# blackjax-devs/blackjax

Measured on NVIDIA B200. Metric: leapfrog-steps/sec (all chains), higher is better.
Workload: dtype f32

## Files before the change

### blackjax_b200/csrc/bjx_dense.cu

```cuda
#include <vector>

#include "bjx_handle.h"
#include "bjx_internal.h"
#include <cuda_fp16.h>

#include "bjx_gemm.h"
#include "bjx_prng.cuh"

using namespace bjx;

namespace bjx {

constexpr int kRowWarps = 8;

__device__ __forceinline__ float wsum(float v) {
#pragma unroll
  for (int o = 16; o > 0; o >>= 1) v += __shfl_xor_sync(0xffffffffu, v, o);
  return v;
}

__device__ __forceinline__ float wmax(float v) {
#pragma unroll
  for (int o = 16; o > 0; o >>= 1) v = fmaxf(v, __shfl_xor_sync(0xffffffffu, v, o));
  return v;
}
__device__ __forceinline__ float max4(float m, float4 v) {
  return fmaxf(fmaxf(m, fmaxf(fabsf(v.x), fabsf(v.y))), fmaxf(fabsf(v.z), fabsf(v.w)));
}

__device__ __forceinline__ void split2(float x, uint16_t& h1, uint16_t& h2) {
  const __half a = __float2half_rn(x);
  const __half b = __float2half_rn(x - __half2float(a));
  h1 = __half_as_ushort(a);
  h2 = __half_as_ushort(b);
}
__device__ __forceinline__ uint2 pack4(const uint16_t (&v)[4]) {
  return make_uint2((uint32_t)v[0] | ((uint32_t)v[1] << 16), (uint32_t)v[2] | ((uint32_t)v[3] << 16));
}
__device__ __forceinline__ void store_planes(uint16_t* row, int KP, int k, float4 v, float sc) {
  uint16_t p1[4], p2[4];
  split2(v.x * sc, p1[0], p2[0]);
  split2(v.y * sc, p1[1], p2[1]);
  split2(v.z * sc, p1[2], p2[2]);
  split2(v.w * sc, p1[3], p2[3]);
  *reinterpret_cast<uint2*>(row + k) = pack4(p1);
  *reinterpret_cast<uint2*>(row + (size_t)KP + k) = pack4(p2);
}

__global__ void k_rows_split2(int R, int K, const float* __restrict__ x, uint16_t* __restrict__ xs, float* __restrict__ unscale,
                              float* __restrict__ rowmax, float* __restrict__ rowmax_zero) {
  const int lane = threadIdx.x & 31, r = blockIdx.x * kRowWarps + (threadIdx.x >> 5);
  if (r >= R) return;
  const float4* xr = reinterpret_cast<const float4*>(x + (size_t)r * K);
  float amax = 0.f;
  for (int i = lane; i < K / 4; i += 32) amax = max4(amax, xr[i]);
  amax = wmax(amax);
  const float sc = pow2_lift(amax);
  const int KP = plane_stride(K);
  uint16_t* row = xs + (size_t)r * 2 * KP;
  for (int i = lane; i < K / 4; i += 32) store_planes(row, KP, 4 * i, xr[i], sc);
  if (lane == 0) {
    unscale[r] = 1.0f / sc;
    if (rowmax) rowmax[r] = amax;
    if (rowmax_zero) rowmax_zero[r] = 0.f;
  }
}

__global__ void k_planes_fixup(int R, int K, const float* __restrict__ y, uint16_t* __restrict__ ys,
                               const float* __restrict__ stale_max, const float* __restrict__ new_max,
                               float* __restrict__ unscale) {
  const int lane = threadIdx.x & 31;
  const int r0 = (blockIdx.x * (blockDim.x >> 5) + (threadIdx.x >> 5)) * 32;
  const int r = r0 + lane;
  asm volatile("griddepcontrol.wait;" ::: "memory");
  bool bad = false;
  if (r < R) {
    const float mx = new_max[r];
    const float t = mx * plane_lift(stale_max[r]);
    bad = (mx > 0.f) && (mx <= 3.0e38f) && !(t >= kPlaneWindowLo && t < kPlaneWindowHi);
  }
  unsigned todo = __ballot_sync(0xffffffffu, bad);
  const int KP = plane_stride(K);
  while (todo) {
    const int rr = r0 + (__ffs(todo) - 1);
    todo &= todo - 1;
    const float sc = pow2_lift(new_max[rr]);
    const float4* xr = reinterpret_cast<const float4*>(y + (size_t)rr * K);
    uint16_t* row = ys + (size_t)rr * 2 * KP;
    for (int i = lane; i < K / 4; i += 32) store_planes(row, KP, 4 * i, xr[i], sc);
    if (lane == 0) unscale[rr] = 1.0f / sc;
  }
}

__global__ void k_absmax(long long n4, const float* __restrict__ x, float* out) {
  float m = 0.f;
  for (long long t = (long long)blockIdx.x * blockDim.x + threadIdx.x; t < n4; t += (long long)gridDim.x * blockDim.x)
    m = max4(m, reinterpret_cast<const float4*>(x)[t]);
  m = wmax(m);
  if ((threadIdx.x & 31) == 0) atomicMax(reinterpret_cast<int*>(out), __float_as_int(m));
}
__global__ void k_matrix_split2(long long R, int K, const float* __restrict__ x, uint16_t* __restrict__ xs,
                                const float* __restrict__ amax, float* __restrict__ unscale) {
  const long long t = (long long)blockIdx.x * blockDim.x + threadIdx.x;
  const float sc = pow2_lift(amax[0]);
  if (t == 0) unscale[0] = 1.0f / sc;
  if (t >= R * K / 4) return;
  const long long e = t * 4;
  const long long r = e / K;
  const int k = (int)(e % K);
  const int KP = plane_stride(K);
  store_planes(xs + r * 2 * KP, KP, k, reinterpret_cast<const float4*>(x)[t], sc);
}

__global__ void k_rows_open(int C, int D, float* __restrict__ p, const float* __restrict__ g, const float* __restrict__ q,
                            float eps, const float* __restrict__ eps_dev, uint16_t* __restrict__ p_planes,
                            float* __restrict__ p_unscale, float* __restrict__ pmax0, float* __restrict__ pmax1,
                            float* __restrict__ qmax0, float* __restrict__ qmax1) {
  const int lane = threadIdx.x & 31, c = blockIdx.x * kRowWarps + (threadIdx.x >> 5);
  if (c >= C) return;
  const size_t ro = (size_t)c * D;
  const float eh = (eps_dev ? eps_dev[c] : eps) * 0.5f;
  float pm = 0.f, qm = 0.f;
  for (int i = lane; i < D / 4; i += 32) {
    float4 pv = __ldcs(reinterpret_cast<const float4*>(p + ro) + i);
    const float4 gv = __ldcs(reinterpret_cast<const float4*>(g + ro) + i);
    pv.x = fmaf(eh, gv.x, pv.x); pv.y = fmaf(eh, gv.y, pv.y); pv.z = fmaf(eh, gv.z, pv.z); pv.w = fmaf(eh, gv.w, pv.w);
    reinterpret_cast<float4*>(p + ro)[i] = pv;
    pm = max4(pm, pv);
    if (q) qm = max4(qm, __ldcs(reinterpret_cast<const float4*>(q + ro) + i));
  }
  pm = wmax(pm);
  qm = wmax(qm);
  const float sc = pow2_lift(pm);
  const int KP = plane_stride(D);
  uint16_t* row = p_planes + (size_t)c * 2 * KP;
  for (int i = lane; i < D / 4; i += 32) store_planes(row, KP, 4 * i, reinterpret_cast<const float4*>(p + ro)[i], sc);
  if (lane == 0) {
    p_unscale[c] = 1.0f / sc;
    pmax0[c] = pm;
    pmax1[c] = 0.f;
    if (q) { qmax0[c] = qm; qmax1[c] = 0.f; }
  }
}

__global__ void k_dense_normal(int C, int D, const uint32_t* __restrict__ keys, float* __restrict__ z, bool split_first,
                               int key_shared, uint32_t chain_offset) {
  const long long t = (long long)blockIdx.x * blockDim.x + threadIdx.x;
  const long long n4 = (long long)C * D / 4;
  if (t >= n4) return;
  const long long e = t * 4;
  const int c = (int)(e / D);
  const uint32_t i = (uint32_t)(e % D);
  Key km = key_shared ? fold_in(Key{keys[0], keys[1]}, chain_offset + (uint32_t)c) : Key{keys[2 * c], keys[2 * c + 1]};
  if (split_first) km = fold_in(km, 0u);
  float4 o;
  o.x = normal_at(km, i);
  o.y = normal_at(km, i + 1);
  o.z = normal_at(km, i + 2);
  o.w = normal_at(km, i + 3);
  reinterpret_cast<float4*>(z)[t] = o;
}

__global__ void k_rows_scale(int C, int D, const float* __restrict__ a, long long a_stride, const float* __restrict__ x,
                             float* __restrict__ y) {
  const long long t = (long long)blockIdx.x * blockDim.x + threadIdx.x;
  const long long n4 = (long long)C * D / 4;
  if (t >= n4) return;
  const long long e = t * 4;
  const int c = (int)(e / D);
  const int i = (int)(e % D);
  const float4 av = *reinterpret_cast<const float4*>(a + (size_t)c * a_stride + i);
  const float4 xv = __ldcs(reinterpret_cast<const float4*>(x) + t);
  __stcs(reinterpret_cast<float4*>(y) + t, make_float4(av.x * xv.x, av.y * xv.y, av.z * xv.z, av.w * xv.w));
}

__global__ void k_rows_axpy(int C, int D, float* __restrict__ x, const float* __restrict__ y, float eps,
                            const float* __restrict__ eps_dev, float coef) {
  const long long t = (long long)blockIdx.x * blockDim.x + threadIdx.x;
  const long long n4 = (long long)C * D / 4;
  if (t >= n4) return;
  const int c = (int)(t * 4 / D);
  const float a = (eps_dev ? eps_dev[c] : eps) * coef;
  float4 xv = __ldcs(reinterpret_cast<const float4*>(x) + t);
  const float4 yv = __ldcs(reinterpret_cast<const float4*>(y) + t);
  xv.x = fmaf(a, yv.x, xv.x); xv.y = fmaf(a, yv.y, xv.y); xv.z = fmaf(a, yv.z, xv.z); xv.w = fmaf(a, yv.w, xv.w);
  __stcs(reinterpret_cast<float4*>(x) + t, xv);
}

__global__ void k_rows_energy(int C, int D, const float* __restrict__ v, const float* __restrict__ p,
                              const float* __restrict__ logp, float* __restrict__ e, float p_sign) {
  const int lane = threadIdx.x & 31, c = blockIdx.x * kRowWarps + (threadIdx.x >> 5);
  if (c >= C) return;
  const float4* vr = reinterpret_cast<const float4*>(v + (size_t)c * D);
  const float4* pr = reinterpret_cast<const float4*>(p + (size_t)c * D);
  float acc = 0.f;
  for (int i = lane; i < D / 4; i += 32) {
    const float4 a = __ldcs(vr + i), b = __ldcs(pr + i);
    acc = fmaf(a.x, b.x, acc); acc = fmaf(a.y, b.y, acc); acc = fmaf(a.z, b.z, acc); acc = fmaf(a.w, b.w, acc);
  }
  acc = wsum(acc);
  if (lane == 0) e[c] = -logp[c] + 0.5f * acc * p_sign;
}

template <int TARGET>
__global__ void k_rows_grad_kick(int C, int D, const float* __restrict__ q, const float* __restrict__ aux,
                                 const float* __restrict__ inv_var, const float* __restrict__ mean, float offset,
                                 float* __restrict__ p, float eps, const float* __restrict__ eps_dev,
                                 float* __restrict__ g_out, float* __restrict__ logp_out, int kicks,
                                 uint16_t* __restrict__ p_split ,
                                 float* __restrict__ p_unscale) {
  const int lane = threadIdx.x & 31, c = blockIdx.x * kRowWarps + (threadIdx.x >> 5);
  if (c >= C) return;
  const size_t ro = (size_t)c * D;
  const float eps_c = eps_dev ? eps_dev[c] : eps;
  const float eh = eps_c * 0.5f;
  float acc = 0.f, amax = 0.f;
  for (int i = lane; i < D / 4; i += 32) {
    const float4 qv = __ldcs(reinterpret_cast<const float4*>(q + ro) + i);
    float4 gv;
    if (TARGET == 2) {
      gv = __ldcs(reinterpret_cast<const float4*>(aux + ro) + i);
      acc = fmaf(qv.x, gv.x, acc); acc = fmaf(qv.y, gv.y, acc); acc = fmaf(qv.z, gv.z, acc); acc = fmaf(qv.w, gv.w, acc);
    } else {
      const float4 w = __ldg(reinterpret_cast<const float4*>(inv_var) + i);
      float4 d = qv;
      if (mean) {
        const float4 m = __ldg(reinterpret_cast<const float4*>(mean) + i);
        d = make_float4(qv.x - m.x, qv.y - m.y, qv.z - m.z, qv.w - m.w);
      }
      gv = make_float4(d.x * -w.x, d.y * -w.y, d.z * -w.z, d.w * -w.w);
      acc = fmaf(d.x, gv.x, acc); acc = fmaf(d.y, gv.y, acc); acc = fmaf(d.z, gv.z, acc); acc = fmaf(d.w, gv.w, acc);
    }
    if (TARGET != 2) __stcs(reinterpret_cast<float4*>(g_out + ro) + i, gv);
    if (p) {
      float4 pv = __ldcs(reinterpret_cast<const float4*>(p + ro) + i);
      pv.x = fmaf(eh, gv.x, pv.x); pv.y = fmaf(eh, gv.y, pv.y); pv.z = fmaf(eh, gv.z, pv.z); pv.w = fmaf(eh, gv.w, pv.w);
      if (kicks == 2) {
        pv.x = fmaf(eh, gv.x, pv.x); pv.y = fmaf(eh, gv.y, pv.y); pv.z = fmaf(eh, gv.z, pv.z); pv.w = fmaf(eh, gv.w, pv.w);
      }
      if (p_split) {
        reinterpret_cast<float4*>(p + ro)[i] = pv;
        amax = max4(amax, pv);
      } else {
        __stcs(reinterpret_cast<float4*>(p + ro) + i, pv);
      }
    }
  }
  if (p_split) {
    const float sc = pow2_lift(wmax(amax));
    const int KP = plane_stride(D);
    uint16_t* row = p_split + (size_t)c * 2 * KP;
    for (int i = lane; i < D / 4; i += 32) store_planes(row, KP, 4 * i, reinterpret_cast<const float4*>(p + ro)[i], sc);
    if (lane == 0) p_unscale[c] = 1.0f / sc;
  }
  acc = wsum(acc);
  if (lane == 0) logp_out[c] = 0.5f * acc + offset;
}

__global__ void k_rows_accept(int C, int D, const uint32_t* __restrict__ keys, const float* __restrict__ e0,
                              const float* __restrict__ e1, float div_thr, const float* __restrict__ qw,
                              const float* __restrict__ gw, const float* __restrict__ lw, const float* q_in,
                              const float* g_in, const float* l_in, float* q_out, float* g_out, float* l_out, int L,
                              InfoPtrs info, int key_shared, uint32_t chain_offset) {
  const int lane = threadIdx.x & 31, c = blockIdx.x * kRowWarps + (threadIdx.x >> 5);
  if (c >= C) return;
  const Key rk = key_shared ? fold_in(Key{keys[0], keys[1]}, chain_offset + (uint32_t)c) : Key{keys[2 * c], keys[2 * c + 1]};
  const Key ki = fold_in(rk, 1u);
  float delta = e0[c] - e1[c];
  if (isnan(delta)) delta = -__int_as_float(0x7f800000);
  const bool is_div = (-delta) > div_thr;
  float pa = expf(delta);
  pa = pa > 1.0f ? 1.0f : pa;
  const bool acc = uniform01(ki) < pa;
  const size_t ro = (size_t)c * D;
  if (acc || q_out != q_in) {
    const float4* sq = reinterpret_cast<const float4*>((acc ? qw : q_in) + ro);
    const float4* sg = reinterpret_cast<const float4*>((acc ? gw : g_in) + ro);
    for (int i = lane; i < D / 4; i += 32) {
      __stcs(reinterpret_cast<float4*>(q_out + ro) + i, __ldcs(sq + i));
      __stcs(reinterpret_cast<float4*>(g_out + ro) + i, __ldcs(sg + i));
    }
    if (lane == 0) l_out[c] = acc ? lw[c] : l_in[c];
  }
  if (lane == 0) {
    if (info.acceptance_rate) info.acceptance_rate[c] = pa;
    if (info.is_accepted) info.is_accepted[c] = acc;
    if (info.is_divergent) info.is_divergent[c] = is_div;
    if (info.energy) info.energy[c] = e1[c];
    if (info.num_integration_steps) info.num_integration_steps[c] = L;
  }
}
}

#define DN_CUDA(call)                                                \
  do {                                                               \
    cudaError_t e_ = (call);                                         \
    if (e_ != cudaSuccess) return bjx_cuda_fail(h, e_, #call);       \
  } while (0)
#define DN_LAUNCH(where)                                             \
  do {                                                               \
    cudaError_t e_ = cudaGetLastError();                             \
    if (e_ != cudaSuccess) return bjx_cuda_fail(h, e_, where);       \
  } while (0)

static inline dim3 g4(long long n4) { return dim3((unsigned)((n4 + 255) / 256)); }
static inline dim3 grow(int C) { return dim3((C + kRowWarps - 1) / kRowWarps); }

struct DenseWs {
  float *p, *v, *q, *g, *lw, *e0, *e1;
  uint16_t* xs[2];
  float* unscale[2];
  float* rmax[2];
  float* mat_max;
  float* mat_unscale;
};
enum { MAT_IMM = 0, MAT_MSQRT = 1, MAT_PREC = 2 };
enum { PL_P = 0, PL_Q = 1 };

constexpr int kParts = 1;
struct Part {
  int c0, n;
  cudaStream_t st;
  int index;
};

static int dense_ws(bjx_handle_t h, DenseWs& w) {
  const size_t C = h->cfg.n_chains, D = h->cfg.dim;
  const size_t row = ((C * D * sizeof(float)) + 255) & ~(size_t)255, vec = ((C * sizeof(float)) + 255) & ~(size_t)255;
  const size_t KP = plane_stride((int)D);
  const size_t xsb = ((C * 2 * KP * sizeof(uint16_t)) + 255) & ~(size_t)255;
  const size_t mat = ((D * 2 * KP * sizeof(uint16_t)) + 255) & ~(size_t)255;
  const size_t need = 4 * row + 11 * vec + 2 * xsb + 3 * mat + 256;
  if (h->dense_bytes < need) {
    if (h->dense_block) DN_CUDA(cudaFree(h->dense_block));
    h->dense_block = nullptr;
    DN_CUDA(cudaMalloc((void**)&h->dense_block, need));
    h->dense_bytes = need;
  }
  if (!h->dense_streams_ready) {
    for (int k = 0; k < 2; ++k) {
      DN_CUDA(cudaStreamCreateWithFlags(&h->dense_stream[k], cudaStreamNonBlocking));
      DN_CUDA(cudaEventCreateWithFlags(&h->dense_join[k], cudaEventDisableTiming));
    }
    DN_CUDA(cudaEventCreateWithFlags(&h->dense_fork, cudaEventDisableTiming));
    DN_CUDA(cudaEventCreateWithFlags(&h->dense_stagger, cudaEventDisableTiming));
    h->dense_streams_ready = true;
  }
  char* b = (char*)h->dense_block;
  w.p = (float*)b; w.v = (float*)(b + row); w.q = (float*)(b + 2 * row); w.g = (float*)(b + 3 * row);
  char* vb = b + 4 * row;
  w.lw = (float*)vb; w.e0 = (float*)(vb + vec); w.e1 = (float*)(vb + 2 * vec);
  w.unscale[PL_P] = (float*)(vb + 3 * vec); w.unscale[PL_Q] = (float*)(vb + 4 * vec);
  w.rmax[PL_P] = (float*)(vb + 5 * vec); w.rmax[PL_Q] = (float*)(vb + 8 * vec);
  char* xb = vb + 11 * vec;
  w.xs[PL_P] = (uint16_t*)xb; w.xs[PL_Q] = (uint16_t*)(xb + xsb);
  for (int m = 0; m < 3; ++m) h->dense_mat_s[m] = (uint16_t*)(xb + 2 * xsb + m * mat);
  w.mat_max = (float*)(xb + 2 * xsb + 3 * mat);
  w.mat_unscale = w.mat_max + 4;
  if (h->dense_bytes_built != need) {
    DN_CUDA(cudaMemsetAsync(vb, 0, 11 * vec + 2 * xsb + 3 * mat, h->stream));
    for (int m = 0; m < 3; ++m) h->dense_mat_src[m] = nullptr;
    h->dense_bytes_built = need;
  }
  const float* src[3] = {h->metric_kind == BJX_METRIC_DENSE ? h->imm : nullptr,
                         h->metric_kind == BJX_METRIC_DENSE ? h->msqrt : nullptr,
                         h->cfg.target.kind == BJX_TARGET_DENSE_GAUSSIAN ? h->cfg.target.precision : nullptr};
  for (int m = 0; m < 3; ++m) {
    if (src[m] && (h->dense_mat_src[m] != src[m] || h->dense_mat_ver[m] != h->dense_version)) {
      DN_CUDA(cudaMemsetAsync(w.mat_max + m, 0, sizeof(float), h->stream));
      k_absmax<<<148, 256, 0, h->stream>>>((long long)D * D / 4, src[m], w.mat_max + m);
      DN_LAUNCH("k_absmax");
      k_matrix_split2<<<g4((long long)D * D / 4), 256, 0, h->stream>>>((long long)D, (int)D, src[m], h->dense_mat_s[m],
                                                                      w.mat_max + m, w.mat_unscale + m);
      DN_LAUNCH("k_matrix_split2");
      h->dense_mat_src[m] = src[m];
      h->dense_mat_ver[m] = h->dense_version;
    }
  }
  return 0;
}

template <class F>
static int for_parts(bjx_handle_t h, F fn) {
  const int C = h->cfg.n_chains;
  const int parts = (C >= 8192) ? kParts : 1;
  if (parts == 1) {
    Part pt{0, C, h->stream, -1};
    return fn(pt);
  }
  DN_CUDA(cudaEventRecord(h->dense_fork, h->stream));
  int rc = 0;
  for (int k = 0; k < parts; ++k) {
    const int c0 = (int)((long long)C * k / parts) & ~255, c1 = (k + 1 == parts) ? C : ((int)((long long)C * (k + 1) / parts) & ~255);
    Part pt{c0, c1 - c0, h->dense_stream[k], k};
    DN_CUDA(cudaStreamWaitEvent(pt.st, h->dense_fork, 0));
    if (rc == 0) rc = fn(pt);
    DN_CUDA(cudaEventRecord(h->dense_join[k], pt.st));
    DN_CUDA(cudaStreamWaitEvent(h->stream, h->dense_join[k], 0));
  }
  return rc;
}

struct PlanesOut {
  int var;
  int phase;
};

static int gemm(bjx_handle_t h, DenseWs& w, const Part& pt, const float* X, int xvar, int mat, float* Y, const float* Cin,
                float alpha, const float* alpha_dev, float beta, bool double_kick = false, PlanesOut po = PlanesOut{-1, 0}) {
  const int D = h->cfg.dim, C = h->cfg.n_chains;
  const size_t ro = (size_t)pt.c0 * D;
  const int KP = plane_stride(D);
  uint16_t* xs = w.xs[xvar] + (size_t)pt.c0 * 2 * KP;
  if (X) {
    k_rows_split2<<<grow(pt.n), kRowWarps * 32, 0, pt.st>>>(pt.n, D, X + ro, xs, w.unscale[xvar] + pt.c0, nullptr, nullptr);
    DN_LAUNCH("k_rows_split2");
  }
  GemmCall g;
  g.x_planes = xs;
  g.a_planes = h->dense_mat_s[mat];
  g.Y = Y + ro;
  g.Cin = Cin ? Cin + ro : nullptr;
  g.planes_out = nullptr;
  g.M = pt.n; g.N = D; g.K = D; g.KP = KP; g.KP_out = KP;
  g.epi.alpha = alpha;
  g.epi.alpha_dev = alpha_dev ? alpha_dev + pt.c0 : nullptr;
  g.epi.x_unscale = w.unscale[xvar] + pt.c0;
  g.epi.mat_unscale = w.mat_unscale + mat;
  g.epi.beta = beta;
  g.epi.has_cin = Cin ? 1 : 0;
  g.epi.double_kick = double_kick ? 1 : 0;
  g.epi.planes = 0;
  g.epi.debug = 0;
  g.epi.out_unscale = nullptr; g.epi.stale_max = nullptr; g.epi.next_max = nullptr; g.epi.zero_max = nullptr;
  if (po.var >= 0) {
    float* ring = w.rmax[po.var];
    g.planes_out = w.xs[po.var] + (size_t)pt.c0 * 2 * KP;
    g.epi.planes = 1;
    g.epi.out_unscale = w.unscale[po.var] + pt.c0;
    g.epi.stale_max = ring + (size_t)(po.phase % 3) * C + pt.c0;
    g.epi.next_max = ring + (size_t)((po.phase + 1) % 3) * C + pt.c0;
    g.epi.zero_max = ring + (size_t)((po.phase + 2) % 3) * C + pt.c0;
  }
  const int rc = gemm_f16x3(g, pt.st);
  if (rc) return bjx_fail(h, BJX_E_UNSUPPORTED, "tensor-core product failed (stage " + std::to_string(rc) + ")");
  if (po.var >= 0) {
    cudaLaunchConfig_t cfg = {};
    cfg.gridDim = dim3((pt.n + 255) / 256);
    cfg.blockDim = dim3(256);
    cfg.stream = pt.st;
    cudaLaunchAttribute attr[1];
    attr[0].id = cudaLaunchAttributeProgrammaticStreamSerialization;
    attr[0].val.programmaticStreamSerializationAllowed = 1;
    cfg.attrs = attr;
    cfg.numAttrs = 1;
    DN_CUDA(cudaLaunchKernelEx(&cfg, k_planes_fixup, pt.n, D, (const float*)(Y + ro), g.planes_out, g.epi.stale_max,
                               (const float*)g.epi.next_max, g.epi.out_unscale));
  }
  return 0;
}

static int dense_velocity(bjx_handle_t h, DenseWs& w, const Part& pt, const float* p, float* v, bool p_presplit = false) {
  const int D = h->cfg.dim;
  if (h->metric_kind == BJX_METRIC_DENSE) return gemm(h, w, pt, p_presplit ? nullptr : p, PL_P, MAT_IMM, v, nullptr, 1.f, nullptr, 0.f);
  const bool per_chain = (h->metric_kind == BJX_METRIC_DIAG_PER_CHAIN);
  const size_t ro = (size_t)pt.c0 * D;
  k_rows_scale<<<g4((long long)pt.n * D / 4), 256, 0, pt.st>>>(pt.n, D, h->imm + (per_chain ? ro : 0), per_chain ? D : 0,
                                                              p + ro, v + ro);
  DN_LAUNCH("k_rows_scale");
  return 0;
}

static int dense_grad(bjx_handle_t h, DenseWs& w, const Part& pt, const float* q, float* p, float eps, const float* eps_dev,
                      float* g, float* logp, int kicks = 1, bool split_p = false, bool q_presplit = false) {
  const int D = h->cfg.dim;
  const bjx_target_desc& t = h->cfg.target;
  const size_t ro = (size_t)pt.c0 * D;
  const float* ed = eps_dev ? eps_dev + pt.c0 : nullptr;
  float* pp = p ? p + ro : nullptr;
  uint16_t* ps = (split_p && pp) ? w.xs[PL_P] + (size_t)pt.c0 * 2 * plane_stride(D) : nullptr;
  if (t.kind == BJX_TARGET_DENSE_GAUSSIAN) {
    int rc = gemm(h, w, pt, q_presplit ? nullptr : q, PL_Q, MAT_PREC, g, nullptr, -1.f, nullptr, 0.f);
    if (rc) return rc;
    k_rows_grad_kick<2><<<grow(pt.n), kRowWarps * 32, 0, pt.st>>>(pt.n, D, q + ro, g + ro, nullptr, nullptr, t.logp_offset,
                                                                pp, eps, ed, g + ro, logp + pt.c0, kicks, ps,
                                                                w.unscale[PL_P] + pt.c0);
  } else if (t.kind == BJX_TARGET_DIAG_GAUSSIAN) {
    k_rows_grad_kick<0><<<grow(pt.n), kRowWarps * 32, 0, pt.st>>>(pt.n, D, q + ro, nullptr, t.inv_var, t.mean, t.logp_offset,
                                                                pp, eps, ed, g + ro, logp + pt.c0, kicks, ps,
                                                                w.unscale[PL_P] + pt.c0);
  } else {
    return bjx_fail(h, BJX_E_UNSUPPORTED, "large-D dense path supports DENSE_GAUSSIAN and DIAG_GAUSSIAN targets");
  }
  DN_LAUNCH("k_rows_grad_kick");
  return 0;
}

static int dense_momentum(bjx_handle_t h, DenseWs& w, const Part& pt, const uint32_t* keys, float* p_out, bool split_first) {
  const int D = h->cfg.dim;
  const size_t ro = (size_t)pt.c0 * D;
  const bool dense_m = (h->metric_kind == BJX_METRIC_DENSE);
  float* z = dense_m ? w.v : p_out;
  const uint32_t* kp = h->key_shared ? keys : keys + 2 * (size_t)pt.c0;
  k_dense_normal<<<g4((long long)pt.n * D / 4), 256, 0, pt.st>>>(pt.n, D, kp, z + ro, split_first, h->key_shared,
                                                                h->chain_offset + (uint32_t)pt.c0);
  DN_LAUNCH("k_dense_normal");
  if (dense_m) return gemm(h, w, pt, z, PL_P, MAT_MSQRT, p_out, nullptr, 1.f, nullptr, 0.f);
  const bool per_chain = (h->metric_kind == BJX_METRIC_DIAG_PER_CHAIN);
  k_rows_scale<<<g4((long long)pt.n * D / 4), 256, 0, pt.st>>>(pt.n, D, h->msqrt + (per_chain ? ro : 0), per_chain ? D : 0,
                                                              z + ro, p_out + ro);
  DN_LAUNCH("k_rows_scale");
  return 0;
}

static int dense_energy(bjx_handle_t h, DenseWs& w, const Part& pt, const float* p, const float* logp, float* e_out,
                        bool p_presplit = false) {
  const int D = h->cfg.dim;
  int rc = dense_velocity(h, w, pt, p, w.v, p_presplit);
  if (rc) return rc;
  const size_t ro = (size_t)pt.c0 * D;
  k_rows_energy<<<grow(pt.n), kRowWarps * 32, 0, pt.st>>>(pt.n, D, w.v + ro, p + ro, logp + pt.c0, e_out + pt.c0, 1.f);
  DN_LAUNCH("k_rows_energy");
  return 0;
}

static int dense_leapfrog_core(bjx_handle_t h, DenseWs& w, const Part& pt, float* q, float* p, float* logp, float* g,
                               float eps, const float* eps_dev, int n_steps, bool p_planes_after = false) {
  const int D = h->cfg.dim, C = h->cfg.n_chains;
  const long long n4 = (long long)pt.n * D / 4;
  const size_t ro = (size_t)pt.c0 * D;
  const float* ed = eps_dev ? eps_dev + pt.c0 : nullptr;
  const bool dense_m = (h->metric_kind == BJX_METRIC_DENSE);
  const bool dense_t = (h->cfg.target.kind == BJX_TARGET_DENSE_GAUSSIAN);
  if (n_steps <= 0) return 0;
  if (dense_m && dense_t) {
    const int KP = plane_stride(D);
    float *pr = w.rmax[PL_P] + pt.c0, *qr = w.rmax[PL_Q] + pt.c0;
    k_rows_open<<<grow(pt.n), kRowWarps * 32, 0, pt.st>>>(pt.n, D, p + ro, g + ro, q + ro, eps, ed,
                                                         w.xs[PL_P] + (size_t)pt.c0 * 2 * KP, w.unscale[PL_P] + pt.c0, pr, pr + C,
                                                         qr, qr + C);
    DN_LAUNCH("k_rows_open");
    int pphase = 0, qphase = 0;
    for (int s = 0; s < n_steps; ++s) {
      int rc = gemm(h, w, pt, nullptr, PL_P, MAT_IMM, q, q, eps_dev ? 1.0f : eps * 1.0f, eps_dev, 1.f, false, PlanesOut{PL_Q, qphase++});
      if (rc) return rc;
      if (s + 1 < n_steps) {
        rc = gemm(h, w, pt, nullptr, PL_Q, MAT_PREC, p, p, eps_dev ? -0.5f : -(eps * 0.5f), eps_dev, 1.f, true, PlanesOut{PL_P, pphase++});
        if (rc) return rc;
      } else {
        rc = dense_grad(h, w, pt, q, p, eps, eps_dev, g, logp, 1, p_planes_after, true);
        if (rc) return rc;
      }
    }
    return 0;
  }
  k_rows_axpy<<<g4(n4), 256, 0, pt.st>>>(pt.n, D, p + ro, g + ro, eps, ed, 0.5f);
  DN_LAUNCH("k_rows_axpy");
  bool p_presplit = false;
  for (int s = 0; s < n_steps; ++s) {
    int rc;
    if (dense_m) {
      rc = gemm(h, w, pt, p_presplit ? nullptr : p, PL_P, MAT_IMM, q, q, eps_dev ? 1.0f : eps * 1.0f, eps_dev, 1.f);
      if (rc) return rc;
    } else {
      rc = dense_velocity(h, w, pt, p, w.v);
      if (rc) return rc;
      k_rows_axpy<<<g4(n4), 256, 0, pt.st>>>(pt.n, D, q + ro, w.v + ro, eps, ed, 1.0f);
      DN_LAUNCH("k_rows_axpy");
    }
    const bool more = (s + 1 < n_steps);
    const bool want_planes = dense_m && (more || p_planes_after);
    rc = dense_grad(h, w, pt, q, p, eps, eps_dev, g, logp, more ? 2 : 1, want_planes);
    if (rc) return rc;
    p_presplit = want_planes;
  }
  return 0;
}

int bjx_dense_velocity(bjx_handle_t h, const float* p, float* v) {
  DenseWs w;
  int rc = dense_ws(h, w);
  if (rc) return rc;
  return for_parts(h, [&](const Part& pt) { return dense_velocity(h, w, pt, p, v); });
}

int bjx_dense_init_state(bjx_handle_t h, const float* q, float* logp_out, float* grad_out) {
  DenseWs w;
  int rc = dense_ws(h, w);
  if (rc) return rc;
  return for_parts(h, [&](const Part& pt) { return dense_grad(h, w, pt, q, nullptr, 0.f, nullptr, grad_out, logp_out); });
}

int bjx_dense_sample_momentum(bjx_handle_t h, const uint32_t* keys, float* p_out, bool split_first) {
  DenseWs w;
  int rc = dense_ws(h, w);
  if (rc) return rc;
  return for_parts(h, [&](const Part& pt) { return dense_momentum(h, w, pt, keys, p_out, split_first); });
}

int bjx_dense_energy(bjx_handle_t h, const float* p, const float* logp, float* e_out) {
  DenseWs w;
  int rc = dense_ws(h, w);
  if (rc) return rc;
  return for_parts(h, [&](const Part& pt) { return dense_energy(h, w, pt, p, logp, e_out); });
}

int bjx_dense_leapfrog(bjx_handle_t h, float* q, float* p, float* logp, float* g, float eps, const float* eps_dev,
                       int n_steps) {
  DenseWs w;
  int rc = dense_ws(h, w);
  if (rc) return rc;
  return for_parts(h, [&](const Part& pt) { return dense_leapfrog_core(h, w, pt, q, p, logp, g, eps, eps_dev, n_steps); });
}

static int dense_hmc_part(bjx_handle_t h, DenseWs& w, const Part& pt, const uint32_t* keys, const float* q_in,
                          const float* logp_in, const float* g_in, float* q_out, float* logp_out, float* g_out, float eps,
                          const float* eps_dev, int L, const InfoPtrs& info) {
  const int D = h->cfg.dim;
  const size_t ro = (size_t)pt.c0 * D;
  const size_t bytes = (size_t)pt.n * D * sizeof(float);
  int rc = dense_momentum(h, w, pt, keys, w.p, true);
  if (rc) return rc;
  if (info.momentum) DN_CUDA(cudaMemcpyAsync(info.momentum + ro, w.p + ro, bytes, cudaMemcpyDeviceToDevice, pt.st));
  rc = dense_energy(h, w, pt, w.p, logp_in, w.e0);
  if (rc) return rc;
  DN_CUDA(cudaMemcpyAsync(w.q + ro, q_in + ro, bytes, cudaMemcpyDeviceToDevice, pt.st));
  DN_CUDA(cudaMemcpyAsync(w.g + ro, g_in + ro, bytes, cudaMemcpyDeviceToDevice, pt.st));
  DN_CUDA(cudaMemcpyAsync(w.lw + pt.c0, logp_in + pt.c0, (size_t)pt.n * sizeof(float), cudaMemcpyDeviceToDevice, pt.st));
  const bool planes_after = (h->metric_kind == BJX_METRIC_DENSE) && L > 0;
  rc = dense_leapfrog_core(h, w, pt, w.q, w.p, w.lw, w.g, eps, eps_dev, L, planes_after);
  if (rc) return rc;
  rc = dense_energy(h, w, pt, w.p, w.lw, w.e1, planes_after);
  if (rc) return rc;
  if (info.proposal_position) DN_CUDA(cudaMemcpyAsync(info.proposal_position + ro, w.q + ro, bytes, cudaMemcpyDeviceToDevice, pt.st));
  if (info.proposal_momentum) {
    DN_CUDA(cudaMemsetAsync(info.proposal_momentum + ro, 0, bytes, pt.st));
    k_rows_axpy<<<g4((long long)pt.n * D / 4), 256, 0, pt.st>>>(pt.n, D, info.proposal_momentum + ro, w.p + ro, -1.0f, nullptr, 1.0f);
    DN_LAUNCH("k_rows_axpy");
  }
  InfoPtrs ip = info;
  if (ip.acceptance_rate) ip.acceptance_rate += pt.c0;
  if (ip.is_accepted) ip.is_accepted += pt.c0;
  if (ip.is_divergent) ip.is_divergent += pt.c0;
  if (ip.energy) ip.energy += pt.c0;
  if (ip.num_integration_steps) ip.num_integration_steps += pt.c0;
  const uint32_t* kp = h->key_shared ? keys : keys + 2 * (size_t)pt.c0;
  k_rows_accept<<<grow(pt.n), kRowWarps * 32, 0, pt.st>>>(pt.n, D, kp, w.e0 + pt.c0, w.e1 + pt.c0, h->cfg.divergence_threshold,
                                                         w.q + ro, w.g + ro, w.lw + pt.c0, q_in + ro, g_in + ro, logp_in + pt.c0,
                                                         q_out + ro, g_out + ro, logp_out + pt.c0, L, ip, h->key_shared,
                                                         h->chain_offset + (uint32_t)pt.c0);
  DN_LAUNCH("k_rows_accept");
  return 0;
}

int bjx_dense_hmc_step(bjx_handle_t h, const uint32_t* keys, const float* q_in, const float* logp_in, const float* g_in,
                       float* q_out, float* logp_out, float* g_out, float eps, const float* eps_dev, int L,
                       const InfoPtrs& info) {
  DenseWs w;
  int rc = dense_ws(h, w);
  if (rc) return rc;
  return for_parts(h, [&](const Part& pt) {
    return dense_hmc_part(h, w, pt, keys, q_in, logp_in, g_in, q_out, logp_out, g_out, eps, eps_dev, L, info);
  });
}

#include "bjx_dense_nuts.cuh"
```

### blackjax_b200/csrc/bjx_dense_nuts.cuh

```cuda
namespace bjx {

struct DnWs {
  float *cq, *cp, *cg, *cv, *cps;
  float *ck_p, *ck_s, *ck_v;
  float *left_v, *right_v;
  float *clogp, *ceps, *sub_weight, *sub_slpa, *sub_logp, *sub_energy, *u_prop;
  int *cn, *cdone, *cdir;
  uint32_t* ctk;
};

__device__ __forceinline__ float dn_dot(const float* a, const float* b, int D, int lane) {
  float acc = 0.f;
  for (int i = lane; i < D / 4; i += 32) {
    const float4 x = reinterpret_cast<const float4*>(a)[i], y = reinterpret_cast<const float4*>(b)[i];
    acc = fmaf(x.x, y.x, acc); acc = fmaf(x.y, y.y, acc); acc = fmaf(x.z, y.z, acc); acc = fmaf(x.w, y.w, acc);
  }
  return wsum(acc);
}
__device__ __forceinline__ void dn_copy(float* dst, const float* src, int D, int lane) {
  for (int i = lane; i < D / 4; i += 32) reinterpret_cast<float4*>(dst)[i] = reinterpret_cast<const float4*>(src)[i];
}
__device__ __forceinline__ void dn_kick(float* p, const float* g, float eh, int D, int lane, uint16_t* planes, float* unscale) {
  float amax = 0.f;
  for (int i = lane; i < D / 4; i += 32) {
    float4 pv = reinterpret_cast<const float4*>(p)[i];
    const float4 gv = reinterpret_cast<const float4*>(g)[i];
    pv.x = fmaf(eh, gv.x, pv.x); pv.y = fmaf(eh, gv.y, pv.y); pv.z = fmaf(eh, gv.z, pv.z); pv.w = fmaf(eh, gv.w, pv.w);
    reinterpret_cast<float4*>(p)[i] = pv;
    amax = max4(amax, pv);
  }
  if (planes) {
    const float sc = pow2_lift(wmax(amax));
    const int KP = plane_stride(D);
    for (int i = lane; i < D / 4; i += 32) store_planes(planes, KP, 4 * i, reinterpret_cast<const float4*>(p)[i], sc);
    if (lane == 0) *unscale = 1.0f / sc;
  }
}
__device__ __forceinline__ bool dn_turning(const float* pl, const float* vl, const float* pr, const float* vr, const float* psum,
                                           const float* sub_a, const float* sub_b, int D, int lane) {
  float al = 0.f, ar = 0.f;
  for (int i = lane; i < D / 4; i += 32) {
    const float4 a = reinterpret_cast<const float4*>(pl)[i], b = reinterpret_cast<const float4*>(pr)[i];
    float4 s = reinterpret_cast<const float4*>(psum)[i];
    if (sub_a) {
      const float4 x = reinterpret_cast<const float4*>(sub_a)[i], y = reinterpret_cast<const float4*>(sub_b)[i];
      s = make_float4(s.x - x.x + y.x, s.y - x.y + y.y, s.z - x.z + y.z, s.w - x.w + y.w);
    }
    const float4 u = reinterpret_cast<const float4*>(vl)[i], w = reinterpret_cast<const float4*>(vr)[i];
    const float r0 = s.x - (b.x + a.x) / 2.0f, r1 = s.y - (b.y + a.y) / 2.0f, r2 = s.z - (b.z + a.z) / 2.0f,
                r3 = s.w - (b.w + a.w) / 2.0f;
    al = fmaf(u.x, r0, al); al = fmaf(u.y, r1, al); al = fmaf(u.z, r2, al); al = fmaf(u.w, r3, al);
    ar = fmaf(w.x, r0, ar); ar = fmaf(w.y, r1, ar); ar = fmaf(w.z, r2, ar); ar = fmaf(w.w, r3, ar);
  }
  al = wsum(al);
  ar = wsum(ar);
  return (al <= 0.f) || (ar <= 0.f);
}

__global__ void k_dn_init(int C, int D, NutsWs ws, DnWs dn, const uint32_t* __restrict__ keys, int key_shared,
                          uint32_t chain_offset, const uint32_t* __restrict__ keyint_override, const float* q_in,
                          const float* logp_in, const float* g_in, float* q_out, float* logp_out, float* g_out, float* mom_out) {
  const int lane = threadIdx.x & 31, c = blockIdx.x * kRowWarps + (threadIdx.x >> 5);
  if (c >= C) return;
  const size_t ro = (size_t)c * D;
  const float kin = 0.5f * dn_dot(dn.left_v + ro, ws.left_p + ro, D, lane);
  dn_copy(ws.right_p + ro, ws.left_p + ro, D, lane);
  dn_copy(dn.right_v + ro, dn.left_v + ro, D, lane);
  dn_copy(ws.psum + ro, ws.left_p + ro, D, lane);
  dn_copy(ws.left_q + ro, q_in + ro, D, lane);
  dn_copy(ws.right_q + ro, q_in + ro, D, lane);
  dn_copy(ws.left_g + ro, g_in + ro, D, lane);
  dn_copy(ws.right_g + ro, g_in + ro, D, lane);
  if (mom_out) dn_copy(mom_out + ro, ws.left_p + ro, D, lane);
  if (q_out != q_in) {
    dn_copy(q_out + ro, q_in + ro, D, lane);
    dn_copy(g_out + ro, g_in + ro, D, lane);
  }
  if (lane == 0) {
    const float logp0 = logp_in[c];
    const float h0 = -logp0 + kin;
    Key ki;
    if (keyint_override) {
      ki = Key{keyint_override[2 * c], keyint_override[2 * c + 1]};
    } else {
      const Key rk = key_shared ? fold_in(Key{keys[0], keys[1]}, chain_offset + (uint32_t)c) : Key{keys[2 * c], keys[2 * c + 1]};
      ki = fold_in(rk, 1u);
    }
    if (q_out != q_in) logp_out[c] = logp0;
    ws.left_logp[c] = logp0;
    ws.right_logp[c] = logp0;
    ws.h0[c] = h0;
    ws.prop_energy[c] = h0;
    ws.prop_weight[c] = 0.f;
    ws.prop_slpa[c] = -__int_as_float(0x7f800000);
    ws.n_states[c] = 0;
    ws.step[c] = 0;
    ws.is_div[c] = 0;
    ws.is_turn[c] = 0;
    ws.key_int[2 * c] = ki.a;
    ws.key_int[2 * c + 1] = ki.b;
  }
}

__global__ void k_dn_begin(int n, int D, int d, NutsWs ws, DnWs dn, const int* __restrict__ list, float eps,
                           const float* __restrict__ eps_dev, uint16_t* __restrict__ p_planes, float* __restrict__ p_unscale) {
  const int lane = threadIdx.x & 31, r = blockIdx.x * kRowWarps + (threadIdx.x >> 5);
  if (r >= n) return;
  const int c = list ? list[r] : r;
  const size_t ro = (size_t)c * D, rr = (size_t)r * D;
  const Key ki{ws.key_int[2 * c], ws.key_int[2 * c + 1]};
  const Key sub = fold_in(ki, (uint32_t)d);
  const int dir = (uniform01(fold_in(sub, 0u)) < 0.5f) ? 1 : -1;
  const Key tk = fold_in(sub, 1u);
  const float ec = (float)dir * (eps_dev ? eps_dev[c] : eps);
  dn_copy(dn.cq + rr, (dir > 0 ? ws.right_q : ws.left_q) + ro, D, lane);
  dn_copy(dn.cp + rr, (dir > 0 ? ws.right_p : ws.left_p) + ro, D, lane);
  dn_copy(dn.cg + rr, (dir > 0 ? ws.right_g : ws.left_g) + ro, D, lane);
  __syncwarp();
  dn_kick(dn.cp + rr, dn.cg + rr, ec * 0.5f, D, lane, p_planes ? p_planes + (size_t)r * 2 * plane_stride(D) : nullptr,
          p_unscale + r);
  if (lane == 0) {
    dn.cdir[r] = dir;
    dn.ceps[r] = ec;
    dn.ctk[2 * r] = tk.a;
    dn.ctk[2 * r + 1] = tk.b;
    dn.u_prop[r] = uniform01(fold_in(sub, 2u));
    dn.cn[r] = 0;
    dn.cdone[r] = 0;
    dn.sub_weight[r] = -__int_as_float(0x7f800000);
    dn.sub_slpa[r] = -__int_as_float(0x7f800000);
    dn.sub_logp[r] = 0.f;
    dn.sub_energy[r] = 0.f;
  }
}

__global__ void k_dn_leaf(int n, int D, int i, int last, int C, NutsWs ws, DnWs dn, const int* __restrict__ list, float div_thr,
                          uint16_t* __restrict__ p_planes, float* __restrict__ p_unscale) {
  const int lane = threadIdx.x & 31, r = blockIdx.x * kRowWarps + (threadIdx.x >> 5);
  if (r >= n) return;
  if (dn.cdone[r]) return;
  const int c = list ? list[r] : r;
  const size_t ro = (size_t)c * D, rr = (size_t)r * D;
  const float* p = dn.cp + rr;
  const float* v = dn.cv + rr;
  float* ps = dn.cps + rr;
  const float logp = dn.clogp[r];
  const float e_new = -logp + 0.5f * dn_dot(v, p, D, lane);
  const float w_new = safe_energy_diff(ws.h0[c], e_new);
  const float slpa_new = fminf(w_new, 0.f);
  const bool is_div = (-w_new) > div_thr;
  float sub_weight = dn.sub_weight[r], sub_slpa = dn.sub_slpa[r];
  bool take;
  if (i == 0) {
    dn_copy(ps, p, D, lane);
    take = true;
    sub_weight = w_new;
    sub_slpa = slpa_new;
  } else {
    for (int k = lane; k < D / 4; k += 32) {
      float4 a = reinterpret_cast<float4*>(ps)[k];
      const float4 b = reinterpret_cast<const float4*>(p)[k];
      a.x = a.x + b.x; a.y = a.y + b.y; a.z = a.z + b.z; a.w = a.w + b.w;
      reinterpret_cast<float4*>(ps)[k] = a;
    }
    const Key tk{dn.ctk[2 * r], dn.ctk[2 * r + 1]};
    const float u_leaf = uniform01(fold_in(tk, (uint32_t)i));
    take = u_leaf < expit_f(w_new - sub_weight);
    sub_weight = logaddexp_f(sub_weight, w_new);
    sub_slpa = logaddexp_f(sub_slpa, slpa_new);
  }
  __syncwarp();
  if (take) {
    dn_copy(ws.sub_prop_q + ro, dn.cq + rr, D, lane);
    dn_copy(ws.sub_prop_g + ro, dn.cg + rr, D, lane);
  }
  const int idx_max = __popc((unsigned)i >> 1);
  const int idx_min = idx_max - __popc((~(unsigned)i & ((unsigned)i + 1u)) - 1u) + 1;
  const size_t lvl = (size_t)C * D;
  if ((i & 1) == 0) {
    dn_copy(dn.ck_p + idx_max * lvl + rr, p, D, lane);
    dn_copy(dn.ck_s + idx_max * lvl + rr, ps, D, lane);
    dn_copy(dn.ck_v + idx_max * lvl + rr, v, D, lane);
  }
  __syncwarp();
  bool turning = false;
  for (int k = idx_max; k >= idx_min && !turning; --k)
    turning = dn_turning(dn.ck_p + k * lvl + rr, dn.ck_v + k * lvl + rr, p, v, ps, dn.ck_s + k * lvl + rr, dn.ck_p + k * lvl + rr,
                         D, lane);
  const bool stop = is_div || turning;
  const int dir = dn.cdir[r];
  if (stop || i == last) {
    dn_copy((dir > 0 ? ws.right_q : ws.left_q) + ro, dn.cq + rr, D, lane);
    dn_copy((dir > 0 ? ws.right_p : ws.left_p) + ro, p, D, lane);
    dn_copy((dir > 0 ? ws.right_g : ws.left_g) + ro, dn.cg + rr, D, lane);
    dn_copy((dir > 0 ? dn.right_v : dn.left_v) + ro, v, D, lane);
  } else {
    __syncwarp();
    dn_kick(dn.cp + rr, dn.cg + rr, dn.ceps[r] * 0.5f, D, lane,
            p_planes ? p_planes + (size_t)r * 2 * plane_stride(D) : nullptr, p_unscale + r);
  }
  if (lane == 0) {
    dn.sub_weight[r] = sub_weight;
    dn.sub_slpa[r] = sub_slpa;
    if (take) {
      dn.sub_logp[r] = logp;
      dn.sub_energy[r] = e_new;
    }
    dn.cn[r] = i + 1;
    if (stop || i == last) {
      if (dir > 0) ws.right_logp[c] = logp; else ws.left_logp[c] = logp;
    }
    if (stop) dn.cdone[r] = is_div ? 1 : 2;
    if (stop && is_div && turning) dn.cdone[r] = 3;
  }
}

__global__ void k_dn_end(int n, int D, int d, int max_doublings, NutsWs ws, DnWs dn, const int* __restrict__ list,
                         int* __restrict__ list_out, int* __restrict__ counter_out, float* q_out, float* logp_out, float* g_out) {
  const int lane = threadIdx.x & 31, r = blockIdx.x * kRowWarps + (threadIdx.x >> 5);
  if (r >= n) return;
  const int c = list ? list[r] : r;
  const size_t ro = (size_t)c * D, rr = (size_t)r * D;
  const int done = dn.cdone[r];
  const bool sub_div = (done & 1) != 0, sub_term = (done & 2) != 0;
  const bool bad = sub_div || sub_term;
  const float sub_weight = dn.sub_weight[r];
  float prop_weight = ws.prop_weight[c];
  bool take2 = false;
  if (!bad) take2 = dn.u_prop[r] < clip_max1(expf(sub_weight - prop_weight));
  if (take2) {
    dn_copy(q_out + ro, ws.sub_prop_q + ro, D, lane);
    dn_copy(g_out + ro, ws.sub_prop_g + ro, D, lane);
  }
  for (int k = lane; k < D / 4; k += 32) {
    float4 a = reinterpret_cast<float4*>(ws.psum + ro)[k];
    const float4 b = reinterpret_cast<const float4*>(dn.cps + rr)[k];
    a.x = a.x + b.x; a.y = a.y + b.y; a.z = a.z + b.z; a.w = a.w + b.w;
    reinterpret_cast<float4*>(ws.psum + ro)[k] = a;
  }
  __syncwarp();
  const bool turning = dn_turning(ws.left_p + ro, dn.left_v + ro, ws.right_p + ro, dn.right_v + ro, ws.psum + ro, nullptr, nullptr,
                                  D, lane);
  const bool is_turn = sub_term || turning;
  const bool run_next = (d + 1 < max_doublings) && !sub_div && !is_turn;
  if (lane == 0) {
    if (!bad) prop_weight = logaddexp_f(prop_weight, sub_weight);
    ws.prop_weight[c] = prop_weight;
    ws.prop_slpa[c] = logaddexp_f(ws.prop_slpa[c], dn.sub_slpa[r]);
    ws.n_states[c] += dn.cn[r];
    ws.step[c] = d + 1;
    if (take2) {
      logp_out[c] = dn.sub_logp[r];
      ws.prop_energy[c] = dn.sub_energy[r];
    }
    ws.is_div[c] = sub_div;
    ws.is_turn[c] = is_turn;
    if (run_next) list_out[atomicAdd(counter_out, 1)] = c;
  }
}

static int dn_ws(bjx_handle_t h, DnWs& dn) {
  const size_t C = h->cfg.n_chains, D = h->cfg.dim, depth = h->cfg.max_tree_depth;
  const size_t row = ((C * D * sizeof(float)) + 255) & ~(size_t)255, vec = ((C * sizeof(float)) + 255) & ~(size_t)255;
  const size_t need = (7 + depth) * row + 12 * vec + 256;
  if (h->dn_bytes < need) {
    if (h->dn_block) DN_CUDA(cudaFree(h->dn_block));
    h->dn_block = nullptr;
    DN_CUDA(cudaMalloc(&h->dn_block, need));
    h->dn_bytes = need;
  }
  char* b = (char*)h->dn_block;
  auto take = [&](size_t bytes) { char* r = b; b += bytes; return r; };
  dn.cq = (float*)take(row); dn.cp = (float*)take(row); dn.cg = (float*)take(row); dn.cv = (float*)take(row);
  dn.cps = (float*)take(row); dn.left_v = (float*)take(row); dn.right_v = (float*)take(row);
  dn.ck_v = (float*)take(depth * row);
  dn.ck_p = h->ws.ckpt_p;
  dn.ck_s = h->ws.ckpt_sum;
  dn.clogp = (float*)take(vec); dn.ceps = (float*)take(vec); dn.sub_weight = (float*)take(vec); dn.sub_slpa = (float*)take(vec);
  dn.sub_logp = (float*)take(vec); dn.sub_energy = (float*)take(vec); dn.u_prop = (float*)take(vec);
  dn.cn = (int*)take(vec); dn.cdone = (int*)take(vec); dn.cdir = (int*)take(vec);
  dn.ctk = (uint32_t*)take(2 * vec);
  return 0;
}

}

using namespace bjx;

int bjx_dense_nuts_step(bjx_handle_t h, const uint32_t* keys, const float* q_in, const float* logp_in, const float* g_in,
                        float* q_out, float* logp_out, float* g_out, float step_size, const float* step_size_dev,
                        int max_num_doublings, InfoPtrs info, const float* momentum_override,
                        const uint32_t* key_integrator_override) {
  DN_CUDA(cudaSetDevice(h->cfg.device));
  const int C = h->cfg.n_chains, D = h->cfg.dim;
  int rc = bjx_ensure_nuts_ws(h);
  if (rc) return rc;
  DenseWs w;
  rc = dense_ws(h, w);
  if (rc) return rc;
  DnWs dn;
  rc = dn_ws(h, dn);
  if (rc) return rc;
  NutsWs& ws = h->ws;
  cudaStream_t st = h->stream;
  const bool dense_m = (h->metric_kind == BJX_METRIC_DENSE);
  Part all{0, C, st, -1};
  DN_CUDA(cudaMemsetAsync(ws.counters, 0, 64 * sizeof(int), st));
  if (momentum_override) {
    DN_CUDA(cudaMemcpyAsync(ws.left_p, momentum_override, (size_t)C * D * sizeof(float), cudaMemcpyDeviceToDevice, st));
  } else {
    rc = dense_momentum(h, w, all, keys, ws.left_p, true);
    if (rc) return rc;
  }
  rc = dense_velocity(h, w, all, ws.left_p, dn.left_v);
  if (rc) return rc;
  k_dn_init<<<grow(C), kRowWarps * 32, 0, st>>>(C, D, ws, dn, keys, h->key_shared, h->chain_offset, key_integrator_override, q_in,
                                                logp_in, g_in, q_out, logp_out, g_out, info.momentum);
  DN_LAUNCH("k_dn_init");

  int n = C;
  const int* list = nullptr;
  int64_t launches = 0;
  for (int d = 0; d < max_num_doublings && n > 0; ++d) {
    Part pt{0, n, st, -1};
    uint16_t* planes = dense_m ? w.xs[PL_P] : nullptr;
    k_dn_begin<<<grow(n), kRowWarps * 32, 0, st>>>(n, D, d, ws, dn, list, step_size, step_size_dev, planes, w.unscale[PL_P]);
    DN_LAUNCH("k_dn_begin");
    const int leaves = 1 << d;
    for (int i = 0; i < leaves; ++i) {
      rc = dense_velocity(h, w, pt, dn.cp, w.v, dense_m);
      if (rc) return rc;
      k_rows_axpy<<<g4((long long)n * D / 4), 256, 0, st>>>(n, D, dn.cq, w.v, 0.f, dn.ceps, 1.0f);
      DN_LAUNCH("k_rows_axpy");
      rc = dense_grad(h, w, pt, dn.cq, dn.cp, 0.f, dn.ceps, dn.cg, dn.clogp, 1, dense_m, false);
      if (rc) return rc;
      rc = dense_velocity(h, w, pt, dn.cp, dn.cv, dense_m);
      if (rc) return rc;
      k_dn_leaf<<<grow(n), kRowWarps * 32, 0, st>>>(n, D, i, leaves - 1, C, ws, dn, list, h->cfg.divergence_threshold, planes,
                                                    w.unscale[PL_P]);
      DN_LAUNCH("k_dn_leaf");
      ++launches;
    }
    int* list_out = (d & 1) ? ws.list_b : ws.list_a;
    k_dn_end<<<grow(n), kRowWarps * 32, 0, st>>>(n, D, d, max_num_doublings, ws, dn, list, list_out, ws.counters + 1 + d, q_out,
                                                 logp_out, g_out);
    DN_LAUNCH("k_dn_end");
    if (d + 1 < max_num_doublings) {
      DN_CUDA(cudaMemcpyAsync(h->h_flag, ws.counters + 1 + d, sizeof(int), cudaMemcpyDeviceToHost, st));
      DN_CUDA(cudaStreamSynchronize(st));
      n = h->h_flag[0];
      list = list_out;
    }
  }
  k_nuts_finish<<<(C + 255) / 256, 256, 0, st>>>(C, ws, info);
  DN_LAUNCH("k_nuts_finish");
  h->last_leaf_launches = launches;
  h->last_depth = -1;
  return 0;
}
```

### blackjax_b200/csrc/bjx_gemm.cu

```cuda
#include <cuda.h>
#include <cuda_fp16.h>
#include <cuda_runtime.h>
#include <stdint.h>

#include <cstdlib>
#include <mutex>

#include "bjx_gemm.h"

namespace bjx {
namespace {

constexpr int kBM = 128;
constexpr int kBN = 256;
constexpr int kUmmaK = 16;
constexpr int kSub = 32;
constexpr int kNSub = kBN / kSub;
constexpr int kThreads = 256;
constexpr uint32_t kTmemCols = 512;
constexpr int kYSlab = 32 * kSub * 4;
constexpr int kPSlab = 32 * kSub * 2;

template <int BK, int STAGES, int NY, int NP>
struct Plan {
  static constexpr int kTileBytes = kBM * BK * 2;
  static constexpr int kStageBytes = 4 * kTileBytes;
  static constexpr int kOffY = STAGES * kStageBytes;
  static constexpr int kOffP = kOffY + 4 * NY * kYSlab;
  static constexpr int kOffBar = kOffP + 4 * NP * 2 * kPSlab;
  static constexpr int kNumBars = 2 * STAGES + 4 + 4 * NY;
  static constexpr int kSmemBytes = kOffBar + kNumBars * 8 + 16 + 1024;
  static_assert(kSmemBytes <= 232448, "over the 227 KB dynamic shared memory limit");
  static_assert(BK == 64 || BK == 32, "one swizzle row per tile row: 128-byte or 64-byte swizzle");
};

__device__ __forceinline__ uint32_t smem_u32(const void* p) { return (uint32_t)__cvta_generic_to_shared(p); }
__device__ __forceinline__ uint32_t cluster_ctarank() {
  uint32_t r;
  asm volatile("mov.u32 %0, %%cluster_ctarank;" : "=r"(r));
  return r;
}
__device__ __forceinline__ uint32_t mapa(uint32_t addr, uint32_t rank) {
  uint32_t r;
  asm volatile("mapa.shared::cluster.u32 %0, %1, %2;" : "=r"(r) : "r"(addr), "r"(rank));
  return r;
}
__device__ __forceinline__ void cluster_sync() {
  asm volatile("barrier.cluster.arrive.release.aligned;\n\tbarrier.cluster.wait.acquire.aligned;" ::: "memory");
}
__device__ __forceinline__ void mbar_init(uint32_t bar, uint32_t count) {
  asm volatile("mbarrier.init.shared::cta.b64 [%0], %1;" ::"r"(bar), "r"(count) : "memory");
}
__device__ __forceinline__ void mbar_wait(uint32_t bar, uint32_t parity) {
  uint32_t done;
  do {
    asm volatile(
        "{\n\t.reg .pred p;\n\t"
        "mbarrier.try_wait.parity.shared::cta.b64 p, [%1], %2;\n\t"
        "selp.u32 %0, 1, 0, p;\n\t}"
        : "=r"(done)
        : "r"(bar), "r"(parity)
        : "memory");
  } while (!done);
}
__device__ __forceinline__ void mbar_wait_cluster(uint32_t bar, uint32_t parity) {
  uint32_t done;
  do {
    asm volatile(
        "{\n\t.reg .pred p;\n\t"
        "mbarrier.try_wait.parity.acquire.cluster.shared::cta.b64 p, [%1], %2;\n\t"
        "selp.u32 %0, 1, 0, p;\n\t}"
        : "=r"(done)
        : "r"(bar), "r"(parity)
        : "memory");
  } while (!done);
}
__device__ __forceinline__ void mbar_expect_tx(uint32_t bar, uint32_t bytes) {
  asm volatile("mbarrier.arrive.expect_tx.shared::cta.b64 _, [%0], %1;" ::"r"(bar), "r"(bytes) : "memory");
}
__device__ __forceinline__ void mbar_arrive_cluster(uint32_t cluster_bar) {
  asm volatile("mbarrier.arrive.release.cluster.shared::cluster.b64 _, [%0];" ::"r"(cluster_bar) : "memory");
}
__device__ __forceinline__ void prefetch_tmap(const CUtensorMap* m) {
  asm volatile("prefetch.tensormap [%0];" ::"l"(reinterpret_cast<uint64_t>(m)) : "memory");
}
__device__ __forceinline__ void tma_load_3d_2sm(uint32_t dst, const CUtensorMap* m, uint32_t leader_bar, int c0, int c1, int c2) {
  asm volatile(
      "cp.async.bulk.tensor.3d.cta_group::2.shared::cluster.global.mbarrier::complete_tx::bytes [%0], [%1, {%3, %4, %5}], [%2];"
      ::"r"(dst), "l"(reinterpret_cast<uint64_t>(m)), "r"(leader_bar), "r"(c0), "r"(c1), "r"(c2)
      : "memory");
}
__device__ __forceinline__ void tma_load_2d(uint32_t dst, const CUtensorMap* m, uint32_t bar, int c0, int c1) {
  asm volatile(
      "cp.async.bulk.tensor.2d.shared::cluster.global.mbarrier::complete_tx::bytes [%0], [%1, {%3, %4}], [%2];"
      ::"r"(dst), "l"(reinterpret_cast<uint64_t>(m)), "r"(bar), "r"(c0), "r"(c1)
      : "memory");
}
__device__ __forceinline__ void tma_store_2d(const CUtensorMap* m, uint32_t src, int c0, int c1) {
  asm volatile("cp.async.bulk.tensor.2d.global.shared::cta.bulk_group [%0, {%2, %3}], [%1];" ::"l"(reinterpret_cast<uint64_t>(m)),
               "r"(src), "r"(c0), "r"(c1)
               : "memory");
}
__device__ __forceinline__ void tma_store_3d(const CUtensorMap* m, uint32_t src, int c0, int c1, int c2) {
  asm volatile("cp.async.bulk.tensor.3d.global.shared::cta.bulk_group [%0, {%2, %3, %4}], [%1];" ::"l"(reinterpret_cast<uint64_t>(m)),
               "r"(src), "r"(c0), "r"(c1), "r"(c2)
               : "memory");
}
__device__ __forceinline__ void tma_store_commit() { asm volatile("cp.async.bulk.commit_group;" ::: "memory"); }
template <int N>
__device__ __forceinline__ void tma_store_wait_read() { asm volatile("cp.async.bulk.wait_group.read %0;" ::"n"(N) : "memory"); }
__device__ __forceinline__ void tma_store_wait_all() { asm volatile("cp.async.bulk.wait_group 0;" ::: "memory"); }
__device__ __forceinline__ void fence_proxy_async() { asm volatile("fence.proxy.async.shared::cta;" ::: "memory"); }
__device__ __forceinline__ void tc_fence_before() { asm volatile("tcgen05.fence::before_thread_sync;" ::: "memory"); }
__device__ __forceinline__ void tc_fence_after() { asm volatile("tcgen05.fence::after_thread_sync;" ::: "memory"); }

__device__ __forceinline__ void umma_f16_2sm(uint32_t tmem_d, uint64_t desc_a, uint64_t desc_b, uint32_t idesc, uint32_t accumulate) {
  asm volatile(
      "{\n\t.reg .pred p;\n\t"
      "setp.ne.b32 p, %4, 0;\n\t"
      "tcgen05.mma.cta_group::2.kind::f16 [%0], %1, %2, %3, p;\n\t}"
      ::"r"(tmem_d), "l"(desc_a), "l"(desc_b), "r"(idesc), "r"(accumulate)
      : "memory");
}
__device__ __forceinline__ void umma_commit_2sm(uint32_t bar) {
  asm volatile("tcgen05.commit.cta_group::2.mbarrier::arrive::one.shared::cluster.multicast::cluster.b64 [%0], %1;" ::"r"(bar),
               "h"((uint16_t)3)
               : "memory");
}
__device__ __forceinline__ void tmem_ld32(uint32_t taddr, uint32_t (&v)[32]) {
  asm volatile(
      "tcgen05.ld.sync.aligned.32x32b.x32.b32 "
      "{%0, %1, %2, %3, %4, %5, %6, %7, %8, %9, %10, %11, %12, %13, %14, %15, "
      "%16, %17, %18, %19, %20, %21, %22, %23, %24, %25, %26, %27, %28, %29, %30, %31}, [%32];"
      : "=r"(v[0]), "=r"(v[1]), "=r"(v[2]), "=r"(v[3]), "=r"(v[4]), "=r"(v[5]), "=r"(v[6]), "=r"(v[7]), "=r"(v[8]), "=r"(v[9]),
        "=r"(v[10]), "=r"(v[11]), "=r"(v[12]), "=r"(v[13]), "=r"(v[14]), "=r"(v[15]), "=r"(v[16]), "=r"(v[17]), "=r"(v[18]),
        "=r"(v[19]), "=r"(v[20]), "=r"(v[21]), "=r"(v[22]), "=r"(v[23]), "=r"(v[24]), "=r"(v[25]), "=r"(v[26]), "=r"(v[27]),
        "=r"(v[28]), "=r"(v[29]), "=r"(v[30]), "=r"(v[31])
      : "r"(taddr)
      : "memory");
}
__device__ __forceinline__ void tmem_ld_wait() { asm volatile("tcgen05.wait::ld.sync.aligned;" ::: "memory"); }
__device__ __forceinline__ float4 lds_f4(uint32_t a) {
  float4 v;
  asm volatile("ld.shared.v4.f32 {%0, %1, %2, %3}, [%4];" : "=f"(v.x), "=f"(v.y), "=f"(v.z), "=f"(v.w) : "r"(a));
  return v;
}
__device__ __forceinline__ void sts_f4(uint32_t a, float4 v) {
  asm volatile("st.shared.v4.f32 [%0], {%1, %2, %3, %4};" ::"r"(a), "f"(v.x), "f"(v.y), "f"(v.z), "f"(v.w) : "memory");
}
__device__ __forceinline__ void sts_u4(uint32_t a, uint32_t x, uint32_t y, uint32_t z, uint32_t w) {
  asm volatile("st.shared.v4.b32 [%0], {%1, %2, %3, %4};" ::"r"(a), "r"(x), "r"(y), "r"(z), "r"(w) : "memory");
}

template <int BK>
__device__ __forceinline__ uint64_t umma_desc(uint32_t smem_addr) {
  const uint32_t lo = ((smem_addr & 0x3FFFFu) >> 4) | (1u << 16);
  const uint32_t hi = ((8u * BK * 2u) >> 4) | (1u << 14) | ((BK == 64 ? 2u : 4u) << 29);
  return (uint64_t)lo | ((uint64_t)hi << 32);
}
constexpr uint32_t kIdesc = (1u << 4) | ((uint32_t)(kBN >> 3) << 17) | ((uint32_t)(256 >> 4) << 24);

__device__ __forceinline__ uint32_t pack_h2(float a, float b) {
  const __half2 h = __floats2half2_rn(a, b);
  return *reinterpret_cast<const uint32_t*>(&h);
}
__device__ __forceinline__ float2 unpack_h2(uint32_t u) { return __half22float2(*reinterpret_cast<const __half2*>(&u)); }

}

__device__ unsigned long long g_gemm_prof[16];
__device__ __forceinline__ unsigned long long clk() {
  unsigned long long t;
  asm volatile("mov.u64 %0, %%clock64;" : "=l"(t));
  return t;
}
#define BJX_PROF_BEGIN(var) unsigned long long var = prof ? clk() : 0ull
#define BJX_PROF_END(var, acc) \
  if (prof) acc += clk() - var

template <int BK, int STAGES, int NY, int NP>
__global__ void __cluster_dims__(2, 1, 1) __launch_bounds__(kThreads, 1)
k_gemm_f16x3(const __grid_constant__ CUtensorMap tm_x,
             const __grid_constant__ CUtensorMap tm_a,
             const __grid_constant__ CUtensorMap tm_c,
             const __grid_constant__ CUtensorMap tm_y,
             const __grid_constant__ CUtensorMap tm_p,
             const GemmEpilogue E, const int M, const int N, const int K, const int tiles_n, const int n_tiles) {
  using P = Plan<BK, STAGES, NY, NP>;
  extern __shared__ uint8_t smem_raw[];
  const uint32_t base = (smem_u32(smem_raw) + 1023u) & ~1023u;
  const uint32_t bar0 = base + P::kOffBar;
  auto full_bar = [&](int s) { return bar0 + 8u * s; };
  auto empty_bar = [&](int s) { return bar0 + 8u * (STAGES + s); };
  auto tfull_bar = [&](int a) { return bar0 + 8u * (2 * STAGES + a); };
  auto tempty_bar = [&](int a) { return bar0 + 8u * (2 * STAGES + 2 + a); };
  auto cin_bar = [&](int q, int slot) { return bar0 + 8u * (2 * STAGES + 4 + q * NY + slot); };
  const uint32_t tmem_slot = bar0 + 8u * P::kNumBars;

  const int warp = threadIdx.x >> 5, lane = threadIdx.x & 31;
  const uint32_t rank = cluster_ctarank();
  const int pair = blockIdx.x >> 1, n_pairs = gridDim.x >> 1;
  const int nkb = (K + BK - 1) / BK;
  const bool prof = (E.debug & 16) != 0;

  if (warp == 0 && lane == 0) {
    prefetch_tmap(&tm_x);
    prefetch_tmap(&tm_a);
    prefetch_tmap(&tm_y);
    if (E.has_cin) prefetch_tmap(&tm_c);
    if (E.planes) prefetch_tmap(&tm_p);
  }
  if (warp == 1 && lane == 0) {
    for (int s = 0; s < STAGES; ++s) {
      mbar_init(full_bar(s), 1);
      mbar_init(empty_bar(s), 1);
    }
    for (int a = 0; a < 2; ++a) {
      mbar_init(tfull_bar(a), 1);
      mbar_init(tempty_bar(a), 8);
    }
    for (int q = 0; q < 4; ++q)
      for (int i = 0; i < NY; ++i) mbar_init(cin_bar(q, i), 1);
    asm volatile("fence.mbarrier_init.release.cluster;" ::: "memory");
  }
  if (warp == 2) {
    asm volatile("tcgen05.alloc.cta_group::2.sync.aligned.shared::cta.b32 [%0], %1;" ::"r"(tmem_slot), "r"(kTmemCols) : "memory");
    asm volatile("tcgen05.relinquish_alloc_permit.cta_group::2.sync.aligned;" ::: "memory");
  }
  tc_fence_before();
  cluster_sync();
  tc_fence_after();
  uint32_t tmem_base;
  asm volatile("ld.shared.u32 %0, [%1];" : "=r"(tmem_base) : "r"(tmem_slot));
  asm volatile("griddepcontrol.wait;" ::: "memory");

  if (warp == 0) {
    if (lane == 0) {
      const uint32_t leader_full0 = mapa(full_bar(0), 0);
      int s = 0;
      uint32_t ph = 0;
      unsigned long long w_empty = 0;
      for (int t = pair; t < n_tiles; t += n_pairs) {
        const int m0 = (t / tiles_n) * (2 * kBM) + (int)rank * kBM;
        const int n0 = (t % tiles_n) * kBN + (int)rank * (kBN / 2);
        for (int kb = 0; kb < nkb; ++kb) {
          BJX_PROF_BEGIN(t0);
          mbar_wait(empty_bar(s), ph ^ 1u);
          BJX_PROF_END(t0, w_empty);
          if (rank == 0) mbar_expect_tx(full_bar(s), 2u * P::kStageBytes);
          const uint32_t st = base + (uint32_t)s * P::kStageBytes;
          const uint32_t fb = leader_full0 + 8u * s;
          tma_load_3d_2sm(st, &tm_x, fb, kb * BK, 0, m0);
          tma_load_3d_2sm(st + 2 * P::kTileBytes, &tm_a, fb, kb * BK, 0, n0);
          tma_load_3d_2sm(st + P::kTileBytes, &tm_x, fb, kb * BK, 1, m0);
          tma_load_3d_2sm(st + 3 * P::kTileBytes, &tm_a, fb, kb * BK, 1, n0);
          if (++s == STAGES) { s = 0; ph ^= 1u; }
        }
      }
      if (prof) atomicAdd(&g_gemm_prof[3], w_empty);
      for (int i = 0; i < STAGES; ++i) {
        mbar_wait(empty_bar(s), ph ^ 1u);
        if (++s == STAGES) { s = 0; ph ^= 1u; }
      }
    }
  } else if (warp == 1) {
    if (rank == 0 && lane == 0) {
      int s = 0, as = 0;
      uint32_t ph = 0, aph = 0;
      unsigned long long w_tempty = 0, w_full = 0;
      BJX_PROF_BEGIN(t_all);
      for (int t = pair; t < n_tiles; t += n_pairs) {
        BJX_PROF_BEGIN(t0);
        mbar_wait_cluster(tempty_bar(as), aph ^ 1u);
        BJX_PROF_END(t0, w_tempty);
        tc_fence_after();
        const uint32_t d = tmem_base + (uint32_t)as * kBN;
        for (int kb = 0; kb < nkb; ++kb) {
          BJX_PROF_BEGIN(t1);
          mbar_wait(full_bar(s), ph);
          BJX_PROF_END(t1, w_full);
          tc_fence_after();
          const uint32_t st = base + (uint32_t)s * P::kStageBytes;
          const uint64_t dx1 = umma_desc<BK>(st), dx2 = umma_desc<BK>(st + P::kTileBytes);
          const uint64_t da1 = umma_desc<BK>(st + 2 * P::kTileBytes), da2 = umma_desc<BK>(st + 3 * P::kTileBytes);
#pragma unroll
          for (int k = 0; k < BK / kUmmaK; ++k)
            umma_f16_2sm(d, dx1 + 2u * k, da1 + 2u * k, kIdesc, (kb | k) != 0);
#pragma unroll
          for (int k = 0; k < BK / kUmmaK; ++k) umma_f16_2sm(d, dx2 + 2u * k, da1 + 2u * k, kIdesc, 1u);
#pragma unroll
          for (int k = 0; k < BK / kUmmaK; ++k) umma_f16_2sm(d, dx1 + 2u * k, da2 + 2u * k, kIdesc, 1u);
          umma_commit_2sm(empty_bar(s));
          if (++s == STAGES) { s = 0; ph ^= 1u; }
        }
        umma_commit_2sm(tfull_bar(as));
        if (++as == 2) { as = 0; aph ^= 1u; }
      }
      if (prof) {
        atomicAdd(&g_gemm_prof[0], w_tempty);
        atomicAdd(&g_gemm_prof[1], w_full);
        atomicAdd(&g_gemm_prof[2], clk() - t_all);
        atomicAdd(&g_gemm_prof[9], 1ull);
      }
    }
  } else if (warp >= 4) {
    const int q = warp & 3;
    const uint32_t ybuf = base + P::kOffY + (uint32_t)q * NY * kYSlab;
    const uint32_t pbuf = base + P::kOffP + (uint32_t)q * NP * 2 * kPSlab;
    const uint32_t leader_tempty0 = mapa(tempty_bar(0), 0);
    const float mat_unscale = E.mat_unscale ? E.mat_unscale[0] : 1.0f;
    const int my_tiles = pair < n_tiles ? (n_tiles - pair + n_pairs - 1) / n_pairs : 0;
    const int n_sub = my_tiles * kNSub;
    const int row_off = (int)rank * kBM + q * 32;
    auto sub_n = [&](int i) { return ((pair + (i / kNSub) * n_pairs) % tiles_n) * kBN + (i % kNSub) * kSub; };
    auto sub_m = [&](int i) { return ((pair + (i / kNSub) * n_pairs) / tiles_n) * (2 * kBM) + row_off; };
    auto load_cin = [&](int i) {
      const uint32_t bar = cin_bar(q, i % NY);
      if (sub_n(i) >= N || (E.debug & 1)) {
        asm volatile("mbarrier.arrive.shared::cta.b64 _, [%0];" ::"r"(bar) : "memory");
        return;
      }
      mbar_expect_tx(bar, kYSlab);
      tma_load_2d(ybuf + (uint32_t)(i % NY) * kYSlab, &tm_c, bar, sub_n(i), sub_m(i));
    };
    constexpr int kAhead = NY - NP;
    if (E.has_cin && lane == 0)
      for (int i = 0; i < kAhead && i < n_sub; ++i) load_cin(i);

    int as = 0;
    uint32_t aph = 0;
    unsigned long long w_tfull = 0, w_cin = 0, w_rd = 0, w_work = 0;
    BJX_PROF_BEGIN(t_all);
    float al = 0.f, sc = 1.f, amax = 0.f;
    int r = 0;
    bool live = false;
    uint32_t tacc = 0;
    for (int i = 0; i < n_sub; ++i) {
      const int j = i % kNSub;
      const int n0s = sub_n(i), m0s = sub_m(i);
      if (lane == 0) {
        BJX_PROF_BEGIN(t0);
        tma_store_wait_read<NP - 1>();
        BJX_PROF_END(t0, w_rd);
        if (E.has_cin && i + kAhead < n_sub) load_cin(i + kAhead);
      }
      __syncwarp();
      if (j == 0) {
        r = m0s + lane;
        live = r < M;
        al = E.alpha;
        if (live) {
          if (E.alpha_dev) al = E.alpha_dev[r] * E.alpha;
          al = al * (E.x_unscale ? E.x_unscale[r] : 1.0f) * mat_unscale;
        }
        sc = 1.0f;
        if (E.planes && live) sc = plane_lift(E.stale_max[r]);
        amax = 0.f;
        BJX_PROF_BEGIN(t0);
        mbar_wait(tfull_bar(as), aph);
        BJX_PROF_END(t0, w_tfull);
        tc_fence_after();
        tacc = tmem_base + (uint32_t)as * kBN + ((uint32_t)(q * 32) << 16);
      }
      uint32_t acc[32];
      tmem_ld32(tacc + (uint32_t)(j * kSub), acc);
      const bool in_cols = n0s < N;
      BJX_PROF_BEGIN(t2);
      if (E.has_cin) mbar_wait(cin_bar(q, i % NY), (uint32_t)((i / NY) & 1));
      BJX_PROF_END(t2, w_cin);
      tmem_ld_wait();
      BJX_PROF_BEGIN(t3);
      if (j == kNSub - 1) {
        tc_fence_before();
        __syncwarp();
        if (lane == 0) mbar_arrive_cluster(leader_tempty0 + 8u * as);
        if (++as == 2) { as = 0; aph ^= 1u; }
      }
      const uint32_t yb = ybuf + (uint32_t)(i % NY) * kYSlab;
      const uint32_t p1b = pbuf + (uint32_t)(i % NP) * 2 * kPSlab, p2b = p1b + kPSlab;
      uint32_t h1lo0 = 0, h1lo1 = 0, h2lo0 = 0, h2lo1 = 0;
      if (!(E.debug & 8))
#pragma unroll
      for (int c = 0; c < 8; ++c) {
        const uint32_t yo = yb + (uint32_t)lane * 128u + (uint32_t)((c ^ (lane & 7)) << 4);
        float4 y;
        const float a0 = __uint_as_float(acc[4 * c]), a1 = __uint_as_float(acc[4 * c + 1]);
        const float a2 = __uint_as_float(acc[4 * c + 2]), a3 = __uint_as_float(acc[4 * c + 3]);
        if (E.has_cin) {
          const float4 cv = lds_f4(yo);
          if (E.double_kick) {
            y.x = fmaf(al, a0, fmaf(al, a0, cv.x));
            y.y = fmaf(al, a1, fmaf(al, a1, cv.y));
            y.z = fmaf(al, a2, fmaf(al, a2, cv.z));
            y.w = fmaf(al, a3, fmaf(al, a3, cv.w));
          } else {
            y.x = fmaf(al, a0, E.beta * cv.x);
            y.y = fmaf(al, a1, E.beta * cv.y);
            y.z = fmaf(al, a2, E.beta * cv.z);
            y.w = fmaf(al, a3, E.beta * cv.w);
          }
        } else {
          y = make_float4(al * a0, al * a1, al * a2, al * a3);
        }
        sts_f4(yo, y);
        if (E.planes) {
          amax = fmaxf(fmaxf(amax, fmaxf(fabsf(y.x), fabsf(y.y))), fmaxf(fabsf(y.z), fabsf(y.w)));
          const float s0 = y.x * sc, s1 = y.y * sc, s2 = y.z * sc, s3 = y.w * sc;
          const uint32_t ha = pack_h2(s0, s1), hb = pack_h2(s2, s3);
          const float2 fa = unpack_h2(ha), fb = unpack_h2(hb);
          const uint32_t ra = pack_h2(s0 - fa.x, s1 - fa.y), rb = pack_h2(s2 - fb.x, s3 - fb.y);
          if ((c & 1) == 0) {
            h1lo0 = ha; h1lo1 = hb; h2lo0 = ra; h2lo1 = rb;
          } else {
            const uint32_t po = (uint32_t)lane * 64u + (uint32_t)(((c >> 1) ^ ((lane >> 1) & 3)) << 4);
            sts_u4(p1b + po, h1lo0, h1lo1, ha, hb);
            sts_u4(p2b + po, h2lo0, h2lo1, ra, rb);
          }
        }
      }
      fence_proxy_async();
      __syncwarp();
      BJX_PROF_END(t3, w_work);
      if (lane == 0 && in_cols) {
        if (!(E.debug & 4)) tma_store_2d(&tm_y, yb, n0s, m0s);
        if (E.planes && !(E.debug & 2)) {
          tma_store_3d(&tm_p, p1b, n0s, 0, m0s);
          tma_store_3d(&tm_p, p2b, n0s, 1, m0s);
        }
        tma_store_commit();
      }
      if (j == kNSub - 1 && E.planes && live) {
        atomicMax(reinterpret_cast<int*>(E.next_max) + r, __float_as_int(amax));
        E.zero_max[r] = 0.f;
        if (n0s < kBN) E.out_unscale[r] = 1.0f / sc;
      }
    }
    if (lane == 0) tma_store_wait_all();
    if (prof && q == 0 && lane == 0) {
      atomicAdd(&g_gemm_prof[4], w_tfull);
      atomicAdd(&g_gemm_prof[5], w_cin);
      atomicAdd(&g_gemm_prof[6], w_rd);
      atomicAdd(&g_gemm_prof[7], w_work);
      atomicAdd(&g_gemm_prof[8], clk() - t_all);
      atomicAdd(&g_gemm_prof[10], 1ull);
    }
  }

  tc_fence_before();
  cluster_sync();
  if (warp == 2) {
    tc_fence_after();
    asm volatile("tcgen05.dealloc.cta_group::2.sync.aligned.b32 %0, %1;" ::"r"(tmem_base), "r"(kTmemCols) : "memory");
  }
}

namespace {
typedef CUresult (*EncodeTiledFn)(CUtensorMap*, CUtensorMapDataType, cuuint32_t, void*, const cuuint64_t*, const cuuint64_t*,
                                  const cuuint32_t*, const cuuint32_t*, CUtensorMapInterleave, CUtensorMapSwizzle,
                                  CUtensorMapL2promotion, CUtensorMapFloatOOBfill);

EncodeTiledFn encode_fn() {
  static EncodeTiledFn fn = nullptr;
  static std::once_flag once;
  std::call_once(once, [] {
    void* p = nullptr;
    cudaDriverEntryPointQueryResult qr;
    if (cudaGetDriverEntryPoint("cuTensorMapEncodeTiled", &p, cudaEnableDefault, &qr) == cudaSuccess &&
        qr == cudaDriverEntryPointSuccess)
      fn = reinterpret_cast<EncodeTiledFn>(p);
  });
  return fn;
}

bool make_plane_map(CUtensorMap* m, const void* ptr, int rows, int K, int KP, int box_k, int box_rows, CUtensorMapSwizzle sw) {
  const cuuint64_t dims[3] = {(cuuint64_t)K, 2, (cuuint64_t)rows};
  const cuuint64_t strides[2] = {(cuuint64_t)KP * 2, (cuuint64_t)KP * 4};
  const cuuint32_t box[3] = {(cuuint32_t)box_k, 1, (cuuint32_t)box_rows};
  const cuuint32_t es[3] = {1, 1, 1};
  return encode_fn()(m, CU_TENSOR_MAP_DATA_TYPE_FLOAT16, 3, const_cast<void*>(ptr), dims, strides, box, es,
                     CU_TENSOR_MAP_INTERLEAVE_NONE, sw, CU_TENSOR_MAP_L2_PROMOTION_L2_256B,
                     CU_TENSOR_MAP_FLOAT_OOB_FILL_NONE) == CUDA_SUCCESS;
}
bool make_row_map(CUtensorMap* m, const void* ptr, int rows, int N) {
  const cuuint64_t dims[2] = {(cuuint64_t)N, (cuuint64_t)rows};
  const cuuint64_t strides[1] = {(cuuint64_t)N * 4};
  const cuuint32_t box[2] = {(cuuint32_t)kSub, 32};
  const cuuint32_t es[2] = {1, 1};
  return encode_fn()(m, CU_TENSOR_MAP_DATA_TYPE_FLOAT32, 2, const_cast<void*>(ptr), dims, strides, box, es,
                     CU_TENSOR_MAP_INTERLEAVE_NONE, CU_TENSOR_MAP_SWIZZLE_128B, CU_TENSOR_MAP_L2_PROMOTION_L2_256B,
                     CU_TENSOR_MAP_FLOAT_OOB_FILL_NONE) == CUDA_SUCCESS;
}

bool pdl_enabled() {
  static const bool on = [] { const char* e = getenv("BJX_GEMM_PDL"); return !(e && e[0] == '0'); }();
  return on;
}

template <int BK, int STAGES, int NY, int NP>
struct Variant {
  using P = Plan<BK, STAGES, NY, NP>;
  static int max_pairs() {
    static int cached = 0;
    static std::once_flag once;
    std::call_once(once, [] {
      int dev = 0, sms = 0;
      cudaGetDevice(&dev);
      cudaDeviceGetAttribute(&sms, cudaDevAttrMultiProcessorCount, dev);
      cudaFuncSetAttribute(k_gemm_f16x3<BK, STAGES, NY, NP>, cudaFuncAttributeMaxDynamicSharedMemorySize, P::kSmemBytes);
      cudaLaunchConfig_t cfg = {};
      cfg.gridDim = dim3(2 * (sms > 0 ? sms : 2));
      cfg.blockDim = dim3(kThreads);
      cfg.dynamicSmemBytes = P::kSmemBytes;
      int n = 0;
      if (cudaOccupancyMaxActiveClusters(&n, k_gemm_f16x3<BK, STAGES, NY, NP>, &cfg) == cudaSuccess && n > 0) cached = n;
      else cached = sms / 2 > 0 ? sms / 2 : 1;
      cudaGetLastError();
    });
    return cached;
  }
  static int run(const GemmCall& g, cudaStream_t stream) {
    CUtensorMap tx, ta, tc, ty, tp;
    const CUtensorMapSwizzle sw = BK == 64 ? CU_TENSOR_MAP_SWIZZLE_128B : CU_TENSOR_MAP_SWIZZLE_64B;
    if (!make_plane_map(&tx, g.x_planes, g.M, g.K, g.KP, BK, kBM, sw)) return 3;
    if (!make_plane_map(&ta, g.a_planes, g.N, g.K, g.KP, BK, kBM, sw)) return 4;
    if (!make_row_map(&ty, g.Y, g.M, g.N)) return 5;
    tc = ty;
    if (g.epi.has_cin && g.Cin != g.Y && !make_row_map(&tc, g.Cin, g.M, g.N)) return 6;
    tp = tx;
    if (g.epi.planes && !make_plane_map(&tp, g.planes_out, g.M, g.N, g.KP_out, kSub, 32, CU_TENSOR_MAP_SWIZZLE_64B)) return 7;
    const int tiles_m = (g.M + 2 * kBM - 1) / (2 * kBM), tiles_n = (g.N + kBN - 1) / kBN;
    const int n_tiles = tiles_m * tiles_n;
    const int pairs = n_tiles < max_pairs() ? n_tiles : max_pairs();
    cudaLaunchConfig_t cfg = {};
    cfg.gridDim = dim3(2 * pairs);
    cfg.blockDim = dim3(kThreads);
    cfg.dynamicSmemBytes = P::kSmemBytes;
    cfg.stream = stream;
    cudaLaunchAttribute attr[1];
    attr[0].id = cudaLaunchAttributeProgrammaticStreamSerialization;
    attr[0].val.programmaticStreamSerializationAllowed = 1;
    cfg.attrs = attr;
    cfg.numAttrs = pdl_enabled() ? 1 : 0;
    const cudaError_t e = cudaLaunchKernelEx(&cfg, k_gemm_f16x3<BK, STAGES, NY, NP>, tx, ta, tc, ty, tp, g.epi, g.M, g.N, g.K,
                                             tiles_n, n_tiles);
    return e == cudaSuccess ? 0 : 8;
  }
};

int variant_id() {
  static int v = [] {
    const char* e = getenv("BJX_GEMM_VARIANT");
    return e ? atoi(e) : 0;
  }();
  return v;
}

}

}
extern "C" int bjx_debug_gemm_counters(unsigned long long* out16, int reset) {
  cudaDeviceSynchronize();
  if (out16 && cudaMemcpyFromSymbol(out16, bjx::g_gemm_prof, sizeof(bjx::g_gemm_prof)) != cudaSuccess) return 1;
  if (reset) {
    unsigned long long z[16] = {0};
    if (cudaMemcpyToSymbol(bjx::g_gemm_prof, z, sizeof(z)) != cudaSuccess) return 2;
  }
  return 0;
}
namespace bjx {

int gemm_f16x3(const GemmCall& g, cudaStream_t stream) {
  if (!encode_fn()) return 1;
  static const int dbg = [] { const char* e = getenv("BJX_GEMM_DEBUG"); return e ? atoi(e) : 0; }();
  if (dbg) const_cast<GemmCall&>(g).epi.debug = dbg;
  if (g.M <= 0 || g.N <= 0 || g.K <= 0 || (g.N & 3) || (g.KP & 7) || (g.KP_out & 7)) return 2;
  switch (variant_id()) {
    case 1: return Variant<64, 2, 4, 2>::run(g, stream);
    case 2: return Variant<32, 5, 3, 1>::run(g, stream);
    case 3: return Variant<64, 3, 1, 1>::run(g, stream);
    default: return Variant<32, 4, 4, 2>::run(g, stream);
  }
}

}
```

### blackjax_b200/csrc/bjx_gemm.h

```cpp
#pragma once
#include <cuda_runtime.h>
#include <stdint.h>

namespace bjx {

__host__ __device__ __forceinline__ int plane_stride(int K) { return (K + 7) & ~7; }

__host__ __device__ __forceinline__ float pow2_lift_to(float amax, int e) {
  if (!(amax > 0.f) || amax > 3.0e38f) return 1.f;
  union { float f; uint32_t u; } b;
  b.f = amax;
  int s = e - ((int)((b.u >> 23) & 0xffu) - 127);
  s = s < -126 ? -126 : (s > 126 ? 126 : s);
  b.u = (uint32_t)(s + 127) << 23;
  return b.f;
}
__host__ __device__ __forceinline__ float pow2_lift(float amax) { return pow2_lift_to(amax, 13); }
__host__ __device__ __forceinline__ float plane_lift(float stale_max) { return pow2_lift_to(stale_max, 6); }
constexpr float kPlaneWindowLo = 0.125f;
constexpr float kPlaneWindowHi = 46340.0f;

struct GemmEpilogue {
  float alpha;
  const float* alpha_dev;
  const float* x_unscale;
  const float* mat_unscale;
  float beta;
  int has_cin;
  int double_kick;
  int planes;
  float* out_unscale;
  const float* stale_max;
  float* next_max;
  float* zero_max;
  int debug;
};

struct GemmCall {
  const uint16_t* x_planes;
  const uint16_t* a_planes;
  float* Y;
  const float* Cin;
  uint16_t* planes_out;
  int M, N, K, KP, KP_out;
  GemmEpilogue epi;
};

int gemm_f16x3(const GemmCall& g, cudaStream_t stream);

}
```

Baseline: 75.33 million.

## Fuse fp16 split of activations into GEMM producer, drop precomputed plane buffers

The GEMM now reads the f32 activation rows directly with a per-row max and splits them into two fp16 planes inside the kernel, instead of separate kernels writing split planes to global memory. The GEMM epilogue no longer emits output planes and no fixup kernel runs; it only records row absmax via atomics. Producer kernels (normal sampling, momentum kick, grad kick) now emit row maxima so the split needs no extra pass. This removes plane writes and reads and several launches, at the cost of in-GEMM conversion work that could slow the mainloop producer.

```diff
diff --git a/blackjax_b200/csrc/bjx_dense.cu b/blackjax_b200/csrc/bjx_dense.cu
--- a/blackjax_b200/csrc/bjx_dense.cu
+++ b/blackjax_b200/csrc/bjx_dense.cu
@@ -47,49 +47,14 @@
   *reinterpret_cast<uint2*>(row + (size_t)KP + k) = pack4(p2);
 }
 
-__global__ void k_rows_split2(int R, int K, const float* __restrict__ x, uint16_t* __restrict__ xs, float* __restrict__ unscale,
-                              float* __restrict__ rowmax, float* __restrict__ rowmax_zero) {
+__global__ void k_rows_max(int R, int K, const float* __restrict__ x, float* __restrict__ rowmax) {
   const int lane = threadIdx.x & 31, r = blockIdx.x * kRowWarps + (threadIdx.x >> 5);
   if (r >= R) return;
   const float4* xr = reinterpret_cast<const float4*>(x + (size_t)r * K);
   float amax = 0.f;
-  for (int i = lane; i < K / 4; i += 32) amax = max4(amax, xr[i]);
+  for (int i = lane; i < K / 4; i += 32) amax = max4(amax, __ldcs(xr + i));
   amax = wmax(amax);
-  const float sc = pow2_lift(amax);
-  const int KP = plane_stride(K);
-  uint16_t* row = xs + (size_t)r * 2 * KP;
-  for (int i = lane; i < K / 4; i += 32) store_planes(row, KP, 4 * i, xr[i], sc);
-  if (lane == 0) {
-    unscale[r] = 1.0f / sc;
-    if (rowmax) rowmax[r] = amax;
-    if (rowmax_zero) rowmax_zero[r] = 0.f;
-  }
-}
-
-__global__ void k_planes_fixup(int R, int K, const float* __restrict__ y, uint16_t* __restrict__ ys,
-                               const float* __restrict__ stale_max, const float* __restrict__ new_max,
-                               float* __restrict__ unscale) {
-  const int lane = threadIdx.x & 31;
-  const int r0 = (blockIdx.x * (blockDim.x >> 5) + (threadIdx.x >> 5)) * 32;
-  const int r = r0 + lane;
-  asm volatile("griddepcontrol.wait;" ::: "memory");
-  bool bad = false;
-  if (r < R) {
-    const float mx = new_max[r];
-    const float t = mx * plane_lift(stale_max[r]);
-    bad = (mx > 0.f) && (mx <= 3.0e38f) && !(t >= kPlaneWindowLo && t < kPlaneWindowHi);
-  }
-  unsigned todo = __ballot_sync(0xffffffffu, bad);
-  const int KP = plane_stride(K);
-  while (todo) {
-    const int rr = r0 + (__ffs(todo) - 1);
-    todo &= todo - 1;
-    const float sc = pow2_lift(new_max[rr]);
-    const float4* xr = reinterpret_cast<const float4*>(y + (size_t)rr * K);
-    uint16_t* row = ys + (size_t)rr * 2 * KP;
-    for (int i = lane; i < K / 4; i += 32) store_planes(row, KP, 4 * i, xr[i], sc);
-    if (lane == 0) unscale[rr] = 1.0f / sc;
-  }
+  if (lane == 0) rowmax[r] = amax;
 }
 
 __global__ void k_absmax(long long n4, const float* __restrict__ x, float* out) {
@@ -112,53 +77,45 @@
   store_planes(xs + r * 2 * KP, KP, k, reinterpret_cast<const float4*>(x)[t], sc);
 }
 
-__global__ void k_rows_open(int C, int D, float* __restrict__ p, const float* __restrict__ g, const float* __restrict__ q,
-                            float eps, const float* __restrict__ eps_dev, uint16_t* __restrict__ p_planes,
-                            float* __restrict__ p_unscale, float* __restrict__ pmax0, float* __restrict__ pmax1,
-                            float* __restrict__ qmax0, float* __restrict__ qmax1) {
+__global__ void k_rows_open(int C, int D, float* __restrict__ p, const float* __restrict__ g, float eps,
+                            const float* __restrict__ eps_dev, float* __restrict__ pmax0, float* __restrict__ pmax1,
+                            float* __restrict__ qmax0) {
   const int lane = threadIdx.x & 31, c = blockIdx.x * kRowWarps + (threadIdx.x >> 5);
   if (c >= C) return;
   const size_t ro = (size_t)c * D;
   const float eh = (eps_dev ? eps_dev[c] : eps) * 0.5f;
-  float pm = 0.f, qm = 0.f;
+  float pm = 0.f;
   for (int i = lane; i < D / 4; i += 32) {
     float4 pv = __ldcs(reinterpret_cast<const float4*>(p + ro) + i);
     const float4 gv = __ldcs(reinterpret_cast<const float4*>(g + ro) + i);
     pv.x = fmaf(eh, gv.x, pv.x); pv.y = fmaf(eh, gv.y, pv.y); pv.z = fmaf(eh, gv.z, pv.z); pv.w = fmaf(eh, gv.w, pv.w);
-    reinterpret_cast<float4*>(p + ro)[i] = pv;
+    __stcs(reinterpret_cast<float4*>(p + ro) + i, pv);
     pm = max4(pm, pv);
-    if (q) qm = max4(qm, __ldcs(reinterpret_cast<const float4*>(q + ro) + i));
   }
   pm = wmax(pm);
-  qm = wmax(qm);
-  const float sc = pow2_lift(pm);
-  const int KP = plane_stride(D);
-  uint16_t* row = p_planes + (size_t)c * 2 * KP;
-  for (int i = lane; i < D / 4; i += 32) store_planes(row, KP, 4 * i, reinterpret_cast<const float4*>(p + ro)[i], sc);
   if (lane == 0) {
-    p_unscale[c] = 1.0f / sc;
     pmax0[c] = pm;
     pmax1[c] = 0.f;
-    if (q) { qmax0[c] = qm; qmax1[c] = 0.f; }
+    qmax0[c] = 0.f;
   }
 }
 
 __global__ void k_dense_normal(int C, int D, const uint32_t* __restrict__ keys, float* __restrict__ z, bool split_first,
-                               int key_shared, uint32_t chain_offset) {
-  const long long t = (long long)blockIdx.x * blockDim.x + threadIdx.x;
-  const long long n4 = (long long)C * D / 4;
-  if (t >= n4) return;
-  const long long e = t * 4;
-  const int c = (int)(e / D);
-  const uint32_t i = (uint32_t)(e % D);
+                               int key_shared, uint32_t chain_offset, float* __restrict__ rowmax) {
+  const int lane = threadIdx.x & 31, c = blockIdx.x * kRowWarps + (threadIdx.x >> 5);
+  if (c >= C) return;
   Key km = key_shared ? fold_in(Key{keys[0], keys[1]}, chain_offset + (uint32_t)c) : Key{keys[2 * c], keys[2 * c + 1]};
   if (split_first) km = fold_in(km, 0u);
-  float4 o;
-  o.x = normal_at(km, i);
-  o.y = normal_at(km, i + 1);
-  o.z = normal_at(km, i + 2);
-  o.w = normal_at(km, i + 3);
-  reinterpret_cast<float4*>(z)[t] = o;
+  float4* zr = reinterpret_cast<float4*>(z + (size_t)c * D);
+  float amax = 0.f;
+  for (int i = lane; i < D / 4; i += 32) {
+    const uint32_t e = 4u * (uint32_t)i;
+    const float4 o = make_float4(normal_at(km, e), normal_at(km, e + 1), normal_at(km, e + 2), normal_at(km, e + 3));
+    zr[i] = o;
+    amax = max4(amax, o);
+  }
+  amax = wmax(amax);
+  if (rowmax && lane == 0) rowmax[c] = amax;
 }
 
 __global__ void k_rows_scale(int C, int D, const float* __restrict__ a, long long a_stride, const float* __restrict__ x,
@@ -207,8 +164,7 @@
                                  const float* __restrict__ inv_var, const float* __restrict__ mean, float offset,
                                  float* __restrict__ p, float eps, const float* __restrict__ eps_dev,
                                  float* __restrict__ g_out, float* __restrict__ logp_out, int kicks,
-                                 uint16_t* __restrict__ p_split ,
-                                 float* __restrict__ p_unscale) {
+                                 float* __restrict__ p_max ) {
   const int lane = threadIdx.x & 31, c = blockIdx.x * kRowWarps + (threadIdx.x >> 5);
   if (c >= C) return;
   const size_t ro = (size_t)c * D;
@@ -238,20 +194,13 @@
       if (kicks == 2) {
         pv.x = fmaf(eh, gv.x, pv.x); pv.y = fmaf(eh, gv.y, pv.y); pv.z = fmaf(eh, gv.z, pv.z); pv.w = fmaf(eh, gv.w, pv.w);
       }
-      if (p_split) {
-        reinterpret_cast<float4*>(p + ro)[i] = pv;
-        amax = max4(amax, pv);
-      } else {
-        __stcs(reinterpret_cast<float4*>(p + ro) + i, pv);
-      }
-    }
-  }
-  if (p_split) {
-    const float sc = pow2_lift(wmax(amax));
-    const int KP = plane_stride(D);
-    uint16_t* row = p_split + (size_t)c * 2 * KP;
-    for (int i = lane; i < D / 4; i += 32) store_planes(row, KP, 4 * i, reinterpret_cast<const float4*>(p + ro)[i], sc);
-    if (lane == 0) p_unscale[c] = 1.0f / sc;
+      __stcs(reinterpret_cast<float4*>(p + ro) + i, pv);
+      amax = max4(amax, pv);
+    }
+  }
+  if (p_max) {
+    amax = wmax(amax);
+    if (lane == 0) p_max[c] = amax;
   }
   acc = wsum(acc);
   if (lane == 0) logp_out[c] = 0.5f * acc + offset;
@@ -308,14 +257,13 @@
 
 struct DenseWs {
   float *p, *v, *q, *g, *lw, *e0, *e1;
-  uint16_t* xs[2];
-  float* unscale[2];
-  float* rmax[2];
+  float* pmax[2];
+  float* qmax[2];
+  float* xmax;
   float* mat_max;
   float* mat_unscale;
 };
 enum { MAT_IMM = 0, MAT_MSQRT = 1, MAT_PREC = 2 };
-enum { PL_P = 0, PL_Q = 1 };
 
 constexpr int kParts = 1;
 struct Part {
@@ -328,9 +276,8 @@
   const size_t C = h->cfg.n_chains, D = h->cfg.dim;
   const size_t row = ((C * D * sizeof(float)) + 255) & ~(size_t)255, vec = ((C * sizeof(float)) + 255) & ~(size_t)255;
   const size_t KP = plane_stride((int)D);
-  const size_t xsb = ((C * 2 * KP * sizeof(uint16_t)) + 255) & ~(size_t)255;
   const size_t mat = ((D * 2 * KP * sizeof(uint16_t)) + 255) & ~(size_t)255;
-  const size_t need = 4 * row + 11 * vec + 2 * xsb + 3 * mat + 256;
+  const size_t need = 4 * row + 8 * vec + 3 * mat + 256;
   if (h->dense_bytes < need) {
     if (h->dense_block) DN_CUDA(cudaFree(h->dense_block));
     h->dense_block = nullptr;
@@ -350,15 +297,15 @@
   w.p = (float*)b; w.v = (float*)(b + row); w.q = (float*)(b + 2 * row); w.g = (float*)(b + 3 * row);
   char* vb = b + 4 * row;
   w.lw = (float*)vb; w.e0 = (float*)(vb + vec); w.e1 = (float*)(vb + 2 * vec);
-  w.unscale[PL_P] = (float*)(vb + 3 * vec); w.unscale[PL_Q] = (float*)(vb + 4 * vec);
-  w.rmax[PL_P] = (float*)(vb + 5 * vec); w.rmax[PL_Q] = (float*)(vb + 8 * vec);
-  char* xb = vb + 11 * vec;
-  w.xs[PL_P] = (uint16_t*)xb; w.xs[PL_Q] = (uint16_t*)(xb + xsb);
-  for (int m = 0; m < 3; ++m) h->dense_mat_s[m] = (uint16_t*)(xb + 2 * xsb + m * mat);
-  w.mat_max = (float*)(xb + 2 * xsb + 3 * mat);
+  w.pmax[0] = (float*)(vb + 3 * vec); w.pmax[1] = (float*)(vb + 4 * vec);
+  w.qmax[0] = (float*)(vb + 5 * vec); w.qmax[1] = (float*)(vb + 6 * vec);
+  w.xmax = (float*)(vb + 7 * vec);
+  char* xb = vb + 8 * vec;
+  for (int m = 0; m < 3; ++m) h->dense_mat_s[m] = (uint16_t*)(xb + m * mat);
+  w.mat_max = (float*)(xb + 3 * mat);
   w.mat_unscale = w.mat_max + 4;
   if (h->dense_bytes_built != need) {
-    DN_CUDA(cudaMemsetAsync(vb, 0, 11 * vec + 2 * xsb + 3 * mat, h->stream));
+    DN_CUDA(cudaMemsetAsync(vb, 0, 8 * vec + 3 * mat, h->stream));
     for (int m = 0; m < 3; ++m) h->dense_mat_src[m] = nullptr;
     h->dense_bytes_built = need;
   }
@@ -401,68 +348,40 @@
   return rc;
 }
 
-struct PlanesOut {
-  int var;
-  int phase;
-};
-
-static int gemm(bjx_handle_t h, DenseWs& w, const Part& pt, const float* X, int xvar, int mat, float* Y, const float* Cin,
-                float alpha, const float* alpha_dev, float beta, bool double_kick = false, PlanesOut po = PlanesOut{-1, 0}) {
-  const int D = h->cfg.dim, C = h->cfg.n_chains;
-  const size_t ro = (size_t)pt.c0 * D;
-  const int KP = plane_stride(D);
-  uint16_t* xs = w.xs[xvar] + (size_t)pt.c0 * 2 * KP;
-  if (X) {
-    k_rows_split2<<<grow(pt.n), kRowWarps * 32, 0, pt.st>>>(pt.n, D, X + ro, xs, w.unscale[xvar] + pt.c0, nullptr, nullptr);
-    DN_LAUNCH("k_rows_split2");
+static int gemm(bjx_handle_t h, DenseWs& w, const Part& pt, const float* X, const float* x_max, int mat, float* Y,
+                const float* Cin, float alpha, const float* alpha_dev, float beta, bool double_kick = false,
+                float* out_max = nullptr, float* clear_max = nullptr) {
+  const int D = h->cfg.dim;
+  const size_t ro = (size_t)pt.c0 * D;
+  if (!x_max) {
+    k_rows_max<<<grow(pt.n), kRowWarps * 32, 0, pt.st>>>(pt.n, D, X + ro, w.xmax + pt.c0);
+    DN_LAUNCH("k_rows_max");
+    x_max = w.xmax;
   }
   GemmCall g;
-  g.x_planes = xs;
+  g.X = X + ro;
+  g.x_max = x_max + pt.c0;
   g.a_planes = h->dense_mat_s[mat];
   g.Y = Y + ro;
   g.Cin = Cin ? Cin + ro : nullptr;
-  g.planes_out = nullptr;
-  g.M = pt.n; g.N = D; g.K = D; g.KP = KP; g.KP_out = KP;
+  g.M = pt.n; g.N = D; g.K = D;
   g.epi.alpha = alpha;
   g.epi.alpha_dev = alpha_dev ? alpha_dev + pt.c0 : nullptr;
-  g.epi.x_unscale = w.unscale[xvar] + pt.c0;
   g.epi.mat_unscale = w.mat_unscale + mat;
   g.epi.beta = beta;
   g.epi.has_cin = Cin ? 1 : 0;
   g.epi.double_kick = double_kick ? 1 : 0;
-  g.epi.planes = 0;
+  g.epi.out_max = out_max ? out_max + pt.c0 : nullptr;
+  g.epi.clear_max = clear_max ? clear_max + pt.c0 : nullptr;
   g.epi.debug = 0;
-  g.epi.out_unscale = nullptr; g.epi.stale_max = nullptr; g.epi.next_max = nullptr; g.epi.zero_max = nullptr;
-  if (po.var >= 0) {
-    float* ring = w.rmax[po.var];
-    g.planes_out = w.xs[po.var] + (size_t)pt.c0 * 2 * KP;
-    g.epi.planes = 1;
-    g.epi.out_unscale = w.unscale[po.var] + pt.c0;
-    g.epi.stale_max = ring + (size_t)(po.phase % 3) * C + pt.c0;
-    g.epi.next_max = ring + (size_t)((po.phase + 1) % 3) * C + pt.c0;
-    g.epi.zero_max = ring + (size_t)((po.phase + 2) % 3) * C + pt.c0;
-  }
   const int rc = gemm_f16x3(g, pt.st);
   if (rc) return bjx_fail(h, BJX_E_UNSUPPORTED, "tensor-core product failed (stage " + std::to_string(rc) + ")");
-  if (po.var >= 0) {
-    cudaLaunchConfig_t cfg = {};
-    cfg.gridDim = dim3((pt.n + 255) / 256);
-    cfg.blockDim = dim3(256);
-    cfg.stream = pt.st;
-    cudaLaunchAttribute attr[1];
-    attr[0].id = cudaLaunchAttributeProgrammaticStreamSerialization;
-    attr[0].val.programmaticStreamSerializationAllowed = 1;
-    cfg.attrs = attr;
-    cfg.numAttrs = 1;
-    DN_CUDA(cudaLaunchKernelEx(&cfg, k_planes_fixup, pt.n, D, (const float*)(Y + ro), g.planes_out, g.epi.stale_max,
-                               (const float*)g.epi.next_max, g.epi.out_unscale));
-  }
-  return 0;
-}
-
-static int dense_velocity(bjx_handle_t h, DenseWs& w, const Part& pt, const float* p, float* v, bool p_presplit = false) {
-  const int D = h->cfg.dim;
-  if (h->metric_kind == BJX_METRIC_DENSE) return gemm(h, w, pt, p_presplit ? nullptr : p, PL_P, MAT_IMM, v, nullptr, 1.f, nullptr, 0.f);
+  return 0;
+}
+
+static int dense_velocity(bjx_handle_t h, DenseWs& w, const Part& pt, const float* p, float* v, const float* p_max = nullptr) {
+  const int D = h->cfg.dim;
+  if (h->metric_kind == BJX_METRIC_DENSE) return gemm(h, w, pt, p, p_max, MAT_IMM, v, nullptr, 1.f, nullptr, 0.f);
   const bool per_chain = (h->metric_kind == BJX_METRIC_DIAG_PER_CHAIN);
   const size_t ro = (size_t)pt.c0 * D;
   k_rows_scale<<<g4((long long)pt.n * D / 4), 256, 0, pt.st>>>(pt.n, D, h->imm + (per_chain ? ro : 0), per_chain ? D : 0,
@@ -472,23 +391,21 @@
 }
 
 static int dense_grad(bjx_handle_t h, DenseWs& w, const Part& pt, const float* q, float* p, float eps, const float* eps_dev,
-                      float* g, float* logp, int kicks = 1, bool split_p = false, bool q_presplit = false) {
+                      float* g, float* logp, int kicks = 1, float* p_max = nullptr, const float* q_max = nullptr) {
   const int D = h->cfg.dim;
   const bjx_target_desc& t = h->cfg.target;
   const size_t ro = (size_t)pt.c0 * D;
   const float* ed = eps_dev ? eps_dev + pt.c0 : nullptr;
   float* pp = p ? p + ro : nullptr;
-  uint16_t* ps = (split_p && pp) ? w.xs[PL_P] + (size_t)pt.c0 * 2 * plane_stride(D) : nullptr;
+  float* pm = (p_max && pp) ? p_max + pt.c0 : nullptr;
   if (t.kind == BJX_TARGET_DENSE_GAUSSIAN) {
-    int rc = gemm(h, w, pt, q_presplit ? nullptr : q, PL_Q, MAT_PREC, g, nullptr, -1.f, nullptr, 0.f);
+    int rc = gemm(h, w, pt, q, q_max, MAT_PREC, g, nullptr, -1.f, nullptr, 0.f);
     if (rc) return rc;
     k_rows_grad_kick<2><<<grow(pt.n), kRowWarps * 32, 0, pt.st>>>(pt.n, D, q + ro, g + ro, nullptr, nullptr, t.logp_offset,
-                                                                pp, eps, ed, g + ro, logp + pt.c0, kicks, ps,
-                                                                w.unscale[PL_P] + pt.c0);
+                                                                pp, eps, ed, g + ro, logp + pt.c0, kicks, pm);
   } else if (t.kind == BJX_TARGET_DIAG_GAUSSIAN) {
     k_rows_grad_kick<0><<<grow(pt.n), kRowWarps * 32, 0, pt.st>>>(pt.n, D, q + ro, nullptr, t.inv_var, t.mean, t.logp_offset,
-                                                                pp, eps, ed, g + ro, logp + pt.c0, kicks, ps,
-                                                                w.unscale[PL_P] + pt.c0);
+                                                                pp, eps, ed, g + ro, logp + pt.c0, kicks, pm);
   } else {
     return bjx_fail(h, BJX_E_UNSUPPORTED, "large-D dense path supports DENSE_GAUSSIAN and DIAG_GAUSSIAN targets");
   }
@@ -502,10 +419,10 @@
   const bool dense_m = (h->metric_kind == BJX_METRIC_DENSE);
   float* z = dense_m ? w.v : p_out;
   const uint32_t* kp = h->key_shared ? keys : keys + 2 * (size_t)pt.c0;
-  k_dense_normal<<<g4((long long)pt.n * D / 4), 256, 0, pt.st>>>(pt.n, D, kp, z + ro, split_first, h->key_shared,
-                                                                h->chain_offset + (uint32_t)pt.c0);
+  k_dense_normal<<<grow(pt.n), kRowWarps * 32, 0, pt.st>>>(pt.n, D, kp, z + ro, split_first, h->key_shared,
+                                                          h->chain_offset + (uint32_t)pt.c0, dense_m ? w.xmax + pt.c0 : nullptr);
   DN_LAUNCH("k_dense_normal");
-  if (dense_m) return gemm(h, w, pt, z, PL_P, MAT_MSQRT, p_out, nullptr, 1.f, nullptr, 0.f);
+  if (dense_m) return gemm(h, w, pt, z, w.xmax, MAT_MSQRT, p_out, nullptr, 1.f, nullptr, 0.f);
   const bool per_chain = (h->metric_kind == BJX_METRIC_DIAG_PER_CHAIN);
   k_rows_scale<<<g4((long long)pt.n * D / 4), 256, 0, pt.st>>>(pt.n, D, h->msqrt + (per_chain ? ro : 0), per_chain ? D : 0,
                                                               z + ro, p_out + ro);
@@ -514,9 +431,9 @@
 }
 
 static int dense_energy(bjx_handle_t h, DenseWs& w, const Part& pt, const float* p, const float* logp, float* e_out,
-                        bool p_presplit = false) {
-  const int D = h->cfg.dim;
-  int rc = dense_velocity(h, w, pt, p, w.v, p_presplit);
+                        const float* p_max = nullptr) {
+  const int D = h->cfg.dim;
+  int rc = dense_velocity(h, w, pt, p, w.v, p_max);
   if (rc) return rc;
   const size_t ro = (size_t)pt.c0 * D;
   k_rows_energy<<<grow(pt.n), kRowWarps * 32, 0, pt.st>>>(pt.n, D, w.v + ro, p + ro, logp + pt.c0, e_out + pt.c0, 1.f);
@@ -525,8 +442,8 @@
 }
 
 static int dense_leapfrog_core(bjx_handle_t h, DenseWs& w, const Part& pt, float* q, float* p, float* logp, float* g,
-                               float eps, const float* eps_dev, int n_steps, bool p_planes_after = false) {
-  const int D = h->cfg.dim, C = h->cfg.n_chains;
+                               float eps, const float* eps_dev, int n_steps, bool p_max_after = false) {
+  const int D = h->cfg.dim;
   const long long n4 = (long long)pt.n * D / 4;
   const size_t ro = (size_t)pt.c0 * D;
   const float* ed = eps_dev ? eps_dev + pt.c0 : nullptr;
@@ -534,21 +451,18 @@
   const bool dense_t = (h->cfg.target.kind == BJX_TARGET_DENSE_GAUSSIAN);
   if (n_steps <= 0) return 0;
   if (dense_m && dense_t) {
-    const int KP = plane_stride(D);
-    float *pr = w.rmax[PL_P] + pt.c0, *qr = w.rmax[PL_Q] + pt.c0;
-    k_rows_open<<<grow(pt.n), kRowWarps * 32, 0, pt.st>>>(pt.n, D, p + ro, g + ro, q + ro, eps, ed,
-                                                         w.xs[PL_P] + (size_t)pt.c0 * 2 * KP, w.unscale[PL_P] + pt.c0, pr, pr + C,
-                                                         qr, qr + C);
+    k_rows_open<<<grow(pt.n), kRowWarps * 32, 0, pt.st>>>(pt.n, D, p + ro, g + ro, eps, ed, w.pmax[0] + pt.c0,
+                                                         w.pmax[1] + pt.c0, w.qmax[0] + pt.c0);
     DN_LAUNCH("k_rows_open");
-    int pphase = 0, qphase = 0;
     for (int s = 0; s < n_steps; ++s) {
-      int rc = gemm(h, w, pt, nullptr, PL_P, MAT_IMM, q, q, eps_dev ? 1.0f : eps * 1.0f, eps_dev, 1.f, false, PlanesOut{PL_Q, qphase++});
+      const int a = s & 1, b = a ^ 1;
+      int rc = gemm(h, w, pt, p, w.pmax[a], MAT_IMM, q, q, eps_dev ? 1.0f : eps * 1.0f, eps_dev, 1.f, false, w.qmax[a], w.qmax[b]);
       if (rc) return rc;
       if (s + 1 < n_steps) {
-        rc = gemm(h, w, pt, nullptr, PL_Q, MAT_PREC, p, p, eps_dev ? -0.5f : -(eps * 0.5f), eps_dev, 1.f, true, PlanesOut{PL_P, pphase++});
+        rc = gemm(h, w, pt, q, w.qmax[a], MAT_PREC, p, p, eps_dev ? -0.5f : -(eps * 0.5f), eps_dev, 1.f, true, w.pmax[b], w.pmax[a]);
         if (rc) return rc;
       } else {
-        rc = dense_grad(h, w, pt, q, p, eps, eps_dev, g, logp, 1, p_planes_after, true);
+        rc = dense_grad(h, w, pt, q, p, eps, eps_dev, g, logp, 1, p_max_after ? w.pmax[0] : nullptr, w.qmax[a]);
         if (rc) return rc;
       }
     }
@@ -556,11 +470,11 @@
   }
   k_rows_axpy<<<g4(n4), 256, 0, pt.st>>>(pt.n, D, p + ro, g + ro, eps, ed, 0.5f);
   DN_LAUNCH("k_rows_axpy");
-  bool p_presplit = false;
+  const float* p_max = nullptr;
   for (int s = 0; s < n_steps; ++s) {
     int rc;
     if (dense_m) {
-      rc = gemm(h, w, pt, p_presplit ? nullptr : p, PL_P, MAT_IMM, q, q, eps_dev ? 1.0f : eps * 1.0f, eps_dev, 1.f);
+      rc = gemm(h, w, pt, p, p_max, MAT_IMM, q, q, eps_dev ? 1.0f : eps * 1.0f, eps_dev, 1.f);
       if (rc) return rc;
     } else {
       rc = dense_velocity(h, w, pt, p, w.v);
@@ -569,10 +483,10 @@
       DN_LAUNCH("k_rows_axpy");
     }
     const bool more = (s + 1 < n_steps);
-    const bool want_planes = dense_m && (more || p_planes_after);
-    rc = dense_grad(h, w, pt, q, p, eps, eps_dev, g, logp, more ? 2 : 1, want_planes);
+    const bool want_max = dense_m && (more || p_max_after);
+    rc = dense_grad(h, w, pt, q, p, eps, eps_dev, g, logp, more ? 2 : 1, want_max ? w.pmax[0] : nullptr);
     if (rc) return rc;
-    p_presplit = want_planes;
+    p_max = want_max ? w.pmax[0] : nullptr;
   }
   return 0;
 }
@@ -627,10 +541,10 @@
   DN_CUDA(cudaMemcpyAsync(w.q + ro, q_in + ro, bytes, cudaMemcpyDeviceToDevice, pt.st));
   DN_CUDA(cudaMemcpyAsync(w.g + ro, g_in + ro, bytes, cudaMemcpyDeviceToDevice, pt.st));
   DN_CUDA(cudaMemcpyAsync(w.lw + pt.c0, logp_in + pt.c0, (size_t)pt.n * sizeof(float), cudaMemcpyDeviceToDevice, pt.st));
-  const bool planes_after = (h->metric_kind == BJX_METRIC_DENSE) && L > 0;
-  rc = dense_leapfrog_core(h, w, pt, w.q, w.p, w.lw, w.g, eps, eps_dev, L, planes_after);
-  if (rc) return rc;
-  rc = dense_energy(h, w, pt, w.p, w.lw, w.e1, planes_after);
+  const bool max_after = (h->metric_kind == BJX_METRIC_DENSE) && L > 0;
+  rc = dense_leapfrog_core(h, w, pt, w.q, w.p, w.lw, w.g, eps, eps_dev, L, max_after);
+  if (rc) return rc;
+  rc = dense_energy(h, w, pt, w.p, w.lw, w.e1, max_after ? w.pmax[0] : nullptr);
   if (rc) return rc;
   if (info.proposal_position) DN_CUDA(cudaMemcpyAsync(info.proposal_position + ro, w.q + ro, bytes, cudaMemcpyDeviceToDevice, pt.st));
   if (info.proposal_momentum) {
diff --git a/blackjax_b200/csrc/bjx_dense_nuts.cuh b/blackjax_b200/csrc/bjx_dense_nuts.cuh
--- a/blackjax_b200/csrc/bjx_dense_nuts.cuh
+++ b/blackjax_b200/csrc/bjx_dense_nuts.cuh
@@ -20,7 +20,7 @@
 __device__ __forceinline__ void dn_copy(float* dst, const float* src, int D, int lane) {
   for (int i = lane; i < D / 4; i += 32) reinterpret_cast<float4*>(dst)[i] = reinterpret_cast<const float4*>(src)[i];
 }
-__device__ __forceinline__ void dn_kick(float* p, const float* g, float eh, int D, int lane, uint16_t* planes, float* unscale) {
+__device__ __forceinline__ void dn_kick(float* p, const float* g, float eh, int D, int lane, float* pmax) {
   float amax = 0.f;
   for (int i = lane; i < D / 4; i += 32) {
     float4 pv = reinterpret_cast<const float4*>(p)[i];
@@ -29,11 +29,9 @@
     reinterpret_cast<float4*>(p)[i] = pv;
     amax = max4(amax, pv);
   }
-  if (planes) {
-    const float sc = pow2_lift(wmax(amax));
-    const int KP = plane_stride(D);
-    for (int i = lane; i < D / 4; i += 32) store_planes(planes, KP, 4 * i, reinterpret_cast<const float4*>(p)[i], sc);
-    if (lane == 0) *unscale = 1.0f / sc;
+  if (pmax) {
+    amax = wmax(amax);
+    if (lane == 0) *pmax = amax;
   }
 }
 __device__ __forceinline__ bool dn_turning(const float* pl, const float* vl, const float* pr, const float* vr, const float* psum,
@@ -103,7 +101,7 @@
 }
 
 __global__ void k_dn_begin(int n, int D, int d, NutsWs ws, DnWs dn, const int* __restrict__ list, float eps,
-                           const float* __restrict__ eps_dev, uint16_t* __restrict__ p_planes, float* __restrict__ p_unscale) {
+                           const float* __restrict__ eps_dev, float* __restrict__ p_max) {
   const int lane = threadIdx.x & 31, r = blockIdx.x * kRowWarps + (threadIdx.x >> 5);
   if (r >= n) return;
   const int c = list ? list[r] : r;
@@ -117,8 +115,7 @@
   dn_copy(dn.cp + rr, (dir > 0 ? ws.right_p : ws.left_p) + ro, D, lane);
   dn_copy(dn.cg + rr, (dir > 0 ? ws.right_g : ws.left_g) + ro, D, lane);
   __syncwarp();
-  dn_kick(dn.cp + rr, dn.cg + rr, ec * 0.5f, D, lane, p_planes ? p_planes + (size_t)r * 2 * plane_stride(D) : nullptr,
-          p_unscale + r);
+  dn_kick(dn.cp + rr, dn.cg + rr, ec * 0.5f, D, lane, p_max ? p_max + r : nullptr);
   if (lane == 0) {
     dn.cdir[r] = dir;
     dn.ceps[r] = ec;
@@ -135,7 +132,7 @@
 }
 
 __global__ void k_dn_leaf(int n, int D, int i, int last, int C, NutsWs ws, DnWs dn, const int* __restrict__ list, float div_thr,
-                          uint16_t* __restrict__ p_planes, float* __restrict__ p_unscale) {
+                          float* __restrict__ p_max) {
   const int lane = threadIdx.x & 31, r = blockIdx.x * kRowWarps + (threadIdx.x >> 5);
   if (r >= n) return;
   if (dn.cdone[r]) return;
@@ -196,8 +193,7 @@
     dn_copy((dir > 0 ? dn.right_v : dn.left_v) + ro, v, D, lane);
   } else {
     __syncwarp();
-    dn_kick(dn.cp + rr, dn.cg + rr, dn.ceps[r] * 0.5f, D, lane,
-            p_planes ? p_planes + (size_t)r * 2 * plane_stride(D) : nullptr, p_unscale + r);
+    dn_kick(dn.cp + rr, dn.cg + rr, dn.ceps[r] * 0.5f, D, lane, p_max ? p_max + r : nullptr);
   }
   if (lane == 0) {
     dn.sub_weight[r] = sub_weight;
@@ -323,21 +319,20 @@
   int64_t launches = 0;
   for (int d = 0; d < max_num_doublings && n > 0; ++d) {
     Part pt{0, n, st, -1};
-    uint16_t* planes = dense_m ? w.xs[PL_P] : nullptr;
-    k_dn_begin<<<grow(n), kRowWarps * 32, 0, st>>>(n, D, d, ws, dn, list, step_size, step_size_dev, planes, w.unscale[PL_P]);
+    float* pmax = dense_m ? w.pmax[0] : nullptr;
+    k_dn_begin<<<grow(n), kRowWarps * 32, 0, st>>>(n, D, d, ws, dn, list, step_size, step_size_dev, pmax);
     DN_LAUNCH("k_dn_begin");
     const int leaves = 1 << d;
     for (int i = 0; i < leaves; ++i) {
-      rc = dense_velocity(h, w, pt, dn.cp, w.v, dense_m);
+      rc = dense_velocity(h, w, pt, dn.cp, w.v, pmax);
       if (rc) return rc;
       k_rows_axpy<<<g4((long long)n * D / 4), 256, 0, st>>>(n, D, dn.cq, w.v, 0.f, dn.ceps, 1.0f);
       DN_LAUNCH("k_rows_axpy");
-      rc = dense_grad(h, w, pt, dn.cq, dn.cp, 0.f, dn.ceps, dn.cg, dn.clogp, 1, dense_m, false);
+      rc = dense_grad(h, w, pt, dn.cq, dn.cp, 0.f, dn.ceps, dn.cg, dn.clogp, 1, pmax);
       if (rc) return rc;
-      rc = dense_velocity(h, w, pt, dn.cp, dn.cv, dense_m);
+      rc = dense_velocity(h, w, pt, dn.cp, dn.cv, pmax);
       if (rc) return rc;
-      k_dn_leaf<<<grow(n), kRowWarps * 32, 0, st>>>(n, D, i, leaves - 1, C, ws, dn, list, h->cfg.divergence_threshold, planes,
-                                                    w.unscale[PL_P]);
+      k_dn_leaf<<<grow(n), kRowWarps * 32, 0, st>>>(n, D, i, leaves - 1, C, ws, dn, list, h->cfg.divergence_threshold, pmax);
       DN_LAUNCH("k_dn_leaf");
       ++launches;
     }
diff --git a/blackjax_b200/csrc/bjx_gemm.cu b/blackjax_b200/csrc/bjx_gemm.cu
--- a/blackjax_b200/csrc/bjx_gemm.cu
+++ b/blackjax_b200/csrc/bjx_gemm.cu
@@ -13,25 +13,26 @@
 
 constexpr int kBM = 128;
 constexpr int kBN = 256;
+constexpr int kBK = 32;
 constexpr int kUmmaK = 16;
 constexpr int kSub = 32;
 constexpr int kNSub = kBN / kSub;
-constexpr int kThreads = 256;
+constexpr int kThreads = 384;
+constexpr int kConvThreads = 128;
 constexpr uint32_t kTmemCols = 512;
 constexpr int kYSlab = 32 * kSub * 4;
-constexpr int kPSlab = 32 * kSub * 2;
-
-template <int BK, int STAGES, int NY, int NP>
+constexpr int kYStoresInFlight = 2;
+constexpr int kTileBytes = kBM * kBK * 2;
+constexpr int kStageBytes = 4 * kTileBytes;
+
+template <int STAGES, int NY>
 struct Plan {
-  static constexpr int kTileBytes = kBM * BK * 2;
-  static constexpr int kStageBytes = 4 * kTileBytes;
   static constexpr int kOffY = STAGES * kStageBytes;
-  static constexpr int kOffP = kOffY + 4 * NY * kYSlab;
-  static constexpr int kOffBar = kOffP + 4 * NP * 2 * kPSlab;
+  static constexpr int kOffBar = kOffY + 4 * NY * kYSlab;
   static constexpr int kNumBars = 2 * STAGES + 4 + 4 * NY;
   static constexpr int kSmemBytes = kOffBar + kNumBars * 8 + 16 + 1024;
   static_assert(kSmemBytes <= 232448, "over the 227 KB dynamic shared memory limit");
-  static_assert(BK == 64 || BK == 32, "one swizzle row per tile row: 128-byte or 64-byte swizzle");
+  static_assert(NY > kYStoresInFlight, "the Cin prefetch needs a free slab");
 };
 
 __device__ __forceinline__ uint32_t smem_u32(const void* p) { return (uint32_t)__cvta_generic_to_shared(p); }
@@ -101,11 +102,6 @@
                "r"(src), "r"(c0), "r"(c1)
                : "memory");
 }
-__device__ __forceinline__ void tma_store_3d(const CUtensorMap* m, uint32_t src, int c0, int c1, int c2) {
-  asm volatile("cp.async.bulk.tensor.3d.global.shared::cta.bulk_group [%0, {%2, %3, %4}], [%1];" ::"l"(reinterpret_cast<uint64_t>(m)),
-               "r"(src), "r"(c0), "r"(c1), "r"(c2)
-               : "memory");
-}
 __device__ __forceinline__ void tma_store_commit() { asm volatile("cp.async.bulk.commit_group;" ::: "memory"); }
 template <int N>
 __device__ __forceinline__ void tma_store_wait_read() { asm volatile("cp.async.bulk.wait_group.read %0;" ::"n"(N) : "memory"); }
@@ -152,12 +148,20 @@
   asm volatile("st.shared.v4.b32 [%0], {%1, %2, %3, %4};" ::"r"(a), "r"(x), "r"(y), "r"(z), "r"(w) : "memory");
 }
 
-template <int BK>
+__device__ __forceinline__ float4 ldg_nc_f4(const float* p) {
+  float4 v;
+  asm volatile("ld.global.nc.L1::no_allocate.v4.f32 {%0, %1, %2, %3}, [%4];"
+               : "=f"(v.x), "=f"(v.y), "=f"(v.z), "=f"(v.w)
+               : "l"(p));
+  return v;
+}
+
 __device__ __forceinline__ uint64_t umma_desc(uint32_t smem_addr) {
   const uint32_t lo = ((smem_addr & 0x3FFFFu) >> 4) | (1u << 16);
-  const uint32_t hi = ((8u * BK * 2u) >> 4) | (1u << 14) | ((BK == 64 ? 2u : 4u) << 29);
+  const uint32_t hi = ((8u * kBK * 2u) >> 4) | (1u << 14) | (4u << 29);
   return (uint64_t)lo | ((uint64_t)hi << 32);
 }
+__device__ __forceinline__ uint32_t swz64(int r, int c) { return (uint32_t)r * 64u + (uint32_t)((c ^ ((r >> 1) & 3)) << 4); }
 constexpr uint32_t kIdesc = (1u << 4) | ((uint32_t)(kBN >> 3) << 17) | ((uint32_t)(256 >> 4) << 24);
 
 __device__ __forceinline__ uint32_t pack_h2(float a, float b) {
@@ -178,15 +182,15 @@
 #define BJX_PROF_END(var, acc) \
   if (prof) acc += clk() - var
 
-template <int BK, int STAGES, int NY, int NP>
+template <int STAGES, int NY>
 __global__ void __cluster_dims__(2, 1, 1) __launch_bounds__(kThreads, 1)
-k_gemm_f16x3(const __grid_constant__ CUtensorMap tm_x,
-             const __grid_constant__ CUtensorMap tm_a,
+k_gemm_f16x3(const __grid_constant__ CUtensorMap tm_a,
              const __grid_constant__ CUtensorMap tm_c,
              const __grid_constant__ CUtensorMap tm_y,
-             const __grid_constant__ CUtensorMap tm_p,
+             const float* __restrict__ X,
+             const float* __restrict__ x_max,
              const GemmEpilogue E, const int M, const int N, const int K, const int tiles_n, const int n_tiles) {
-  using P = Plan<BK, STAGES, NY, NP>;
+  using P = Plan<STAGES, NY>;
   extern __shared__ uint8_t smem_raw[];
   const uint32_t base = (smem_u32(smem_raw) + 1023u) & ~1023u;
   const uint32_t bar0 = base + P::kOffBar;
@@ -200,19 +204,18 @@
   const int warp = threadIdx.x >> 5, lane = threadIdx.x & 31;
   const uint32_t rank = cluster_ctarank();
   const int pair = blockIdx.x >> 1, n_pairs = gridDim.x >> 1;
-  const int nkb = (K + BK - 1) / BK;
+  const int nkb = (K + kBK - 1) / kBK;
+  const int my_tiles = pair < n_tiles ? (n_tiles - pair + n_pairs - 1) / n_pairs : 0;
   const bool prof = (E.debug & 16) != 0;
 
   if (warp == 0 && lane == 0) {
-    prefetch_tmap(&tm_x);
     prefetch_tmap(&tm_a);
     prefetch_tmap(&tm_y);
     if (E.has_cin) prefetch_tmap(&tm_c);
-    if (E.planes) prefetch_tmap(&tm_p);
   }
   if (warp == 1 && lane == 0) {
     for (int s = 0; s < STAGES; ++s) {
-      mbar_init(full_bar(s), 1);
+      mbar_init(full_bar(s), 1 + 2 * kConvThreads / 32);
       mbar_init(empty_bar(s), 1);
     }
     for (int a = 0; a < 2; ++a) {
@@ -241,19 +244,16 @@
       uint32_t ph = 0;
       unsigned long long w_empty = 0;
       for (int t = pair; t < n_tiles; t += n_pairs) {
-        const int m0 = (t / tiles_n) * (2 * kBM) + (int)rank * kBM;
         const int n0 = (t % tiles_n) * kBN + (int)rank * (kBN / 2);
         for (int kb = 0; kb < nkb; ++kb) {
           BJX_PROF_BEGIN(t0);
           mbar_wait(empty_bar(s), ph ^ 1u);
           BJX_PROF_END(t0, w_empty);
-          if (rank == 0) mbar_expect_tx(full_bar(s), 2u * P::kStageBytes);
-          const uint32_t st = base + (uint32_t)s * P::kStageBytes;
+          if (rank == 0) mbar_expect_tx(full_bar(s), 2u * 2u * kTileBytes);
+          const uint32_t st = base + (uint32_t)s * kStageBytes;
           const uint32_t fb = leader_full0 + 8u * s;
-          tma_load_3d_2sm(st, &tm_x, fb, kb * BK, 0, m0);
-          tma_load_3d_2sm(st + 2 * P::kTileBytes, &tm_a, fb, kb * BK, 0, n0);
-          tma_load_3d_2sm(st + P::kTileBytes, &tm_x, fb, kb * BK, 1, m0);
-          tma_load_3d_2sm(st + 3 * P::kTileBytes, &tm_a, fb, kb * BK, 1, n0);
+          tma_load_3d_2sm(st + 2 * kTileBytes, &tm_a, fb, kb * kBK, 0, n0);
+          tma_load_3d_2sm(st + 3 * kTileBytes, &tm_a, fb, kb * kBK, 1, n0);
           if (++s == STAGES) { s = 0; ph ^= 1u; }
         }
       }
@@ -277,19 +277,19 @@
         const uint32_t d = tmem_base + (uint32_t)as * kBN;
         for (int kb = 0; kb < nkb; ++kb) {
           BJX_PROF_BEGIN(t1);
-          mbar_wait(full_bar(s), ph);
+          mbar_wait_cluster(full_bar(s), ph);
           BJX_PROF_END(t1, w_full);
           tc_fence_after();
-          const uint32_t st = base + (uint32_t)s * P::kStageBytes;
-          const uint64_t dx1 = umma_desc<BK>(st), dx2 = umma_desc<BK>(st + P::kTileBytes);
-          const uint64_t da1 = umma_desc<BK>(st + 2 * P::kTileBytes), da2 = umma_desc<BK>(st + 3 * P::kTileBytes);
+          const uint32_t st = base + (uint32_t)s * kStageBytes;
+          const uint64_t dx1 = umma_desc(st), dx2 = umma_desc(st + kTileBytes);
+          const uint64_t da1 = umma_desc(st + 2 * kTileBytes), da2 = umma_desc(st + 3 * kTileBytes);
 #pragma unroll
-          for (int k = 0; k < BK / kUmmaK; ++k)
+          for (int k = 0; k < kBK / kUmmaK; ++k)
             umma_f16_2sm(d, dx1 + 2u * k, da1 + 2u * k, kIdesc, (kb | k) != 0);
 #pragma unroll
-          for (int k = 0; k < BK / kUmmaK; ++k) umma_f16_2sm(d, dx2 + 2u * k, da1 + 2u * k, kIdesc, 1u);
+          for (int k = 0; k < kBK / kUmmaK; ++k) umma_f16_2sm(d, dx2 + 2u * k, da1 + 2u * k, kIdesc, 1u);
 #pragma unroll
-          for (int k = 0; k < BK / kUmmaK; ++k) umma_f16_2sm(d, dx1 + 2u * k, da2 + 2u * k, kIdesc, 1u);
+          for (int k = 0; k < kBK / kUmmaK; ++k) umma_f16_2sm(d, dx1 + 2u * k, da2 + 2u * k, kIdesc, 1u);
           umma_commit_2sm(empty_bar(s));
           if (++s == STAGES) { s = 0; ph ^= 1u; }
         }
@@ -303,13 +303,69 @@
         atomicAdd(&g_gemm_prof[9], 1ull);
       }
     }
+  } else if (warp >= 8) {
+    const int ct = threadIdx.x - 256;
+    const int chunk = ct & 3, row0 = ct >> 2;
+    const uint32_t leader_full0 = mapa(full_bar(0), 0);
+    const int total = my_tiles * nkb;
+    struct Blk {
+      float4 v[4][2];
+      float m[4];
+    };
+    auto fetch = [&](int i, Blk& b) {
+      const int t = pair + (i / nkb) * n_pairs, kb = i % nkb;
+      const int m0 = (t / tiles_n) * (2 * kBM) + (int)rank * kBM;
+      const int k = kb * kBK + chunk * 8;
+#pragma unroll
+      for (int j = 0; j < 4; ++j) {
+        const int r = m0 + row0 + 32 * j;
+        const float* src = X + (size_t)r * K + k;
+        const bool live = r < M;
+        b.m[j] = live ? __ldg(x_max + r) : 0.f;
+        b.v[j][0] = (live && k < K) ? ldg_nc_f4(src) : make_float4(0.f, 0.f, 0.f, 0.f);
+        b.v[j][1] = (live && k + 4 < K) ? ldg_nc_f4(src + 4) : make_float4(0.f, 0.f, 0.f, 0.f);
+      }
+    };
+    auto put = [&](int i, const Blk& b) {
+      const int s = i % STAGES;
+      mbar_wait(empty_bar(s), (uint32_t)((i / STAGES) & 1) ^ 1u);
+      const uint32_t st = base + (uint32_t)s * kStageBytes;
+#pragma unroll
+      for (int j = 0; j < 4; ++j) {
+        const float sc = pow2_lift(b.m[j]);
+        const float4 a = b.v[j][0], c = b.v[j][1];
+        const float x[8] = {a.x * sc, a.y * sc, a.z * sc, a.w * sc, c.x * sc, c.y * sc, c.z * sc, c.w * sc};
+        uint32_t h1[4], h2[4];
+#pragma unroll
+        for (int e = 0; e < 4; ++e) {
+          h1[e] = pack_h2(x[2 * e], x[2 * e + 1]);
+          const float2 f = unpack_h2(h1[e]);
+          h2[e] = pack_h2(x[2 * e] - f.x, x[2 * e + 1] - f.y);
+        }
+        const uint32_t o = swz64(row0 + 32 * j, chunk);
+        sts_u4(st + o, h1[0], h1[1], h1[2], h1[3]);
+        sts_u4(st + kTileBytes + o, h2[0], h2[1], h2[2], h2[3]);
+      }
+      fence_proxy_async();
+      __syncwarp();
+      if (lane == 0) mbar_arrive_cluster(leader_full0 + 8u * s);
+    };
+    Blk b0, b1;
+    if (total > 0) fetch(0, b0);
+    if (total > 1) fetch(1, b1);
+    for (int i = 0; i < total; i += 2) {
+      put(i, b0);
+      if (i + 2 < total) fetch(i + 2, b0);
+      if (i + 1 < total) {
+        put(i + 1, b1);
+        if (i + 3 < total) fetch(i + 3, b1);
+      }
+    }
   } else if (warp >= 4) {
     const int q = warp & 3;
     const uint32_t ybuf = base + P::kOffY + (uint32_t)q * NY * kYSlab;
-    const uint32_t pbuf = base + P::kOffP + (uint32_t)q * NP * 2 * kPSlab;
     const uint32_t leader_tempty0 = mapa(tempty_bar(0), 0);
     const float mat_unscale = E.mat_unscale ? E.mat_unscale[0] : 1.0f;
-    const int my_tiles = pair < n_tiles ? (n_tiles - pair + n_pairs - 1) / n_pairs : 0;
     const int n_sub = my_tiles * kNSub;
     const int row_off = (int)rank * kBM + q * 32;
     auto sub_n = [&](int i) { return ((pair + (i / kNSub) * n_pairs) % tiles_n) * kBN + (i % kNSub) * kSub; };
@@ -323,7 +379,7 @@
       mbar_expect_tx(bar, kYSlab);
       tma_load_2d(ybuf + (uint32_t)(i % NY) * kYSlab, &tm_c, bar, sub_n(i), sub_m(i));
     };
-    constexpr int kAhead = NY - NP;
+    constexpr int kAhead = NY - kYStoresInFlight;
     if (E.has_cin && lane == 0)
       for (int i = 0; i < kAhead && i < n_sub; ++i) load_cin(i);
 
@@ -331,7 +387,7 @@
     uint32_t aph = 0;
     unsigned long long w_tfull = 0, w_cin = 0, w_rd = 0, w_work = 0;
     BJX_PROF_BEGIN(t_all);
-    float al = 0.f, sc = 1.f, amax = 0.f;
+    float al = 0.f, amax = 0.f;
     int r = 0;
     bool live = false;
     uint32_t tacc = 0;
@@ -340,7 +396,7 @@
       const int n0s = sub_n(i), m0s = sub_m(i);
       if (lane == 0) {
         BJX_PROF_BEGIN(t0);
-        tma_store_wait_read<NP - 1>();
+        tma_store_wait_read<kYStoresInFlight - 1>();
         BJX_PROF_END(t0, w_rd);
         if (E.has_cin && i + kAhead < n_sub) load_cin(i + kAhead);
       }
@@ -351,10 +407,8 @@
         al = E.alpha;
         if (live) {
           if (E.alpha_dev) al = E.alpha_dev[r] * E.alpha;
-          al = al * (E.x_unscale ? E.x_unscale[r] : 1.0f) * mat_unscale;
+          al = al * (1.0f / pow2_lift(x_max[r])) * mat_unscale;
         }
-        sc = 1.0f;
-        if (E.planes && live) sc = plane_lift(E.stale_max[r]);
         amax = 0.f;
         BJX_PROF_BEGIN(t0);
         mbar_wait(tfull_bar(as), aph);
@@ -377,8 +431,6 @@
         if (++as == 2) { as = 0; aph ^= 1u; }
       }
       const uint32_t yb = ybuf + (uint32_t)(i % NY) * kYSlab;
-      const uint32_t p1b = pbuf + (uint32_t)(i % NP) * 2 * kPSlab, p2b = p1b + kPSlab;
-      uint32_t h1lo0 = 0, h1lo1 = 0, h2lo0 = 0, h2lo1 = 0;
       if (!(E.debug & 8))
 #pragma unroll
       for (int c = 0; c < 8; ++c) {
@@ -403,36 +455,18 @@
           y = make_float4(al * a0, al * a1, al * a2, al * a3);
         }
         sts_f4(yo, y);
-        if (E.planes) {
-          amax = fmaxf(fmaxf(amax, fmaxf(fabsf(y.x), fabsf(y.y))), fmaxf(fabsf(y.z), fabsf(y.w)));
-          const float s0 = y.x * sc, s1 = y.y * sc, s2 = y.z * sc, s3 = y.w * sc;
-          const uint32_t ha = pack_h2(s0, s1), hb = pack_h2(s2, s3);
-          const float2 fa = unpack_h2(ha), fb = unpack_h2(hb);
-          const uint32_t ra = pack_h2(s0 - fa.x, s1 - fa.y), rb = pack_h2(s2 - fb.x, s3 - fb.y);
-          if ((c & 1) == 0) {
-            h1lo0 = ha; h1lo1 = hb; h2lo0 = ra; h2lo1 = rb;
-          } else {
-            const uint32_t po = (uint32_t)lane * 64u + (uint32_t)(((c >> 1) ^ ((lane >> 1) & 3)) << 4);
-            sts_u4(p1b + po, h1lo0, h1lo1, ha, hb);
-            sts_u4(p2b + po, h2lo0, h2lo1, ra, rb);
-          }
-        }
+        if (E.out_max && in_cols) amax = fmaxf(fmaxf(amax, fmaxf(fabsf(y.x), fabsf(y.y))), fmaxf(fabsf(y.z), fabsf(y.w)));
       }
       fence_proxy_async();
       __syncwarp();
       BJX_PROF_END(t3, w_work);
-      if (lane == 0 && in_cols) {
-        if (!(E.debug & 4)) tma_store_2d(&tm_y, yb, n0s, m0s);
-        if (E.planes && !(E.debug & 2)) {
-          tma_store_3d(&tm_p, p1b, n0s, 0, m0s);
-          tma_store_3d(&tm_p, p2b, n0s, 1, m0s);
-        }
+      if (lane == 0) {
+        if (in_cols && !(E.debug & 4)) tma_store_2d(&tm_y, yb, n0s, m0s);
         tma_store_commit();
       }
-      if (j == kNSub - 1 && E.planes && live) {
-        atomicMax(reinterpret_cast<int*>(E.next_max) + r, __float_as_int(amax));
-        E.zero_max[r] = 0.f;
-        if (n0s < kBN) E.out_unscale[r] = 1.0f / sc;
+      if (j == kNSub - 1 && E.out_max && live) {
+        atomicMax(reinterpret_cast<int*>(E.out_max) + r, __float_as_int(amax));
+        if (E.clear_max) E.clear_max[r] = 0.f;
       }
     }
     if (lane == 0) tma_store_wait_all();
@@ -496,9 +530,9 @@
   return on;
 }
 
-template <int BK, int STAGES, int NY, int NP>
+template <int STAGES, int NY>
 struct Variant {
-  using P = Plan<BK, STAGES, NY, NP>;
+  using P = Plan<STAGES, NY>;
   static int max_pairs() {
     static int cached = 0;
     static std::once_flag once;
@@ -506,28 +540,24 @@
       int dev = 0, sms = 0;
       cudaGetDevice(&dev);
       cudaDeviceGetAttribute(&sms, cudaDevAttrMultiProcessorCount, dev);
-      cudaFuncSetAttribute(k_gemm_f16x3<BK, STAGES, NY, NP>, cudaFuncAttributeMaxDynamicSharedMemorySize, P::kSmemBytes);
+      cudaFuncSetAttribute(k_gemm_f16x3<STAGES, NY>, cudaFuncAttributeMaxDynamicSharedMemorySize, P::kSmemBytes);
       cudaLaunchConfig_t cfg = {};
       cfg.gridDim = dim3(2 * (sms > 0 ? sms : 2));
       cfg.blockDim = dim3(kThreads);
       cfg.dynamicSmemBytes = P::kSmemBytes;
       int n = 0;
-      if (cudaOccupancyMaxActiveClusters(&n, k_gemm_f16x3<BK, STAGES, NY, NP>, &cfg) == cudaSuccess && n > 0) cached = n;
+      if (cudaOccupancyMaxActiveClusters(&n, k_gemm_f16x3<STAGES, NY>, &cfg) == cudaSuccess && n > 0) cached = n;
       else cached = sms / 2 > 0 ? sms / 2 : 1;
       cudaGetLastError();
     });
     return cached;
   }
   static int run(const GemmCall& g, cudaStream_t stream) {
-    CUtensorMap tx, ta, tc, ty, tp;
-    const CUtensorMapSwizzle sw = BK == 64 ? CU_TENSOR_MAP_SWIZZLE_128B : CU_TENSOR_MAP_SWIZZLE_64B;
-    if (!make_plane_map(&tx, g.x_planes, g.M, g.K, g.KP, BK, kBM, sw)) return 3;
-    if (!make_plane_map(&ta, g.a_planes, g.N, g.K, g.KP, BK, kBM, sw)) return 4;
+    CUtensorMap ta, tc, ty;
+    if (!make_plane_map(&ta, g.a_planes, g.N, g.K, plane_stride(g.K), kBK, kBM, CU_TENSOR_MAP_SWIZZLE_64B)) return 4;
     if (!make_row_map(&ty, g.Y, g.M, g.N)) return 5;
     tc = ty;
     if (g.epi.has_cin && g.Cin != g.Y && !make_row_map(&tc, g.Cin, g.M, g.N)) return 6;
-    tp = tx;
-    if (g.epi.planes && !make_plane_map(&tp, g.planes_out, g.M, g.N, g.KP_out, kSub, 32, CU_TENSOR_MAP_SWIZZLE_64B)) return 7;
     const int tiles_m = (g.M + 2 * kBM - 1) / (2 * kBM), tiles_n = (g.N + kBN - 1) / kBN;
     const int n_tiles = tiles_m * tiles_n;
     const int pairs = n_tiles < max_pairs() ? n_tiles : max_pairs();
@@ -541,7 +571,7 @@
     attr[0].val.programmaticStreamSerializationAllowed = 1;
     cfg.attrs = attr;
     cfg.numAttrs = pdl_enabled() ? 1 : 0;
-    const cudaError_t e = cudaLaunchKernelEx(&cfg, k_gemm_f16x3<BK, STAGES, NY, NP>, tx, ta, tc, ty, tp, g.epi, g.M, g.N, g.K,
+    const cudaError_t e = cudaLaunchKernelEx(&cfg, k_gemm_f16x3<STAGES, NY>, ta, tc, ty, g.X, g.x_max, g.epi, g.M, g.N, g.K,
                                              tiles_n, n_tiles);
     return e == cudaSuccess ? 0 : 8;
   }
@@ -573,13 +603,11 @@
   if (!encode_fn()) return 1;
   static const int dbg = [] { const char* e = getenv("BJX_GEMM_DEBUG"); return e ? atoi(e) : 0; }();
   if (dbg) const_cast<GemmCall&>(g).epi.debug = dbg;
-  if (g.M <= 0 || g.N <= 0 || g.K <= 0 || (g.N & 3) || (g.KP & 7) || (g.KP_out & 7)) return 2;
+  if (g.M <= 0 || g.N <= 0 || g.K <= 0 || (g.N & 3) || (g.K & 3) || !g.X || !g.x_max) return 2;
   switch (variant_id()) {
-    case 1: return Variant<64, 2, 4, 2>::run(g, stream);
-    case 2: return Variant<32, 5, 3, 1>::run(g, stream);
-    case 3: return Variant<64, 3, 1, 1>::run(g, stream);
-    default: return Variant<32, 4, 4, 2>::run(g, stream);
-  }
-}
-
-}
+    case 1: return Variant<5, 4>::run(g, stream);
+    default: return Variant<4, 4>::run(g, stream);
+  }
+}
+
+}
diff --git a/blackjax_b200/csrc/bjx_gemm.h b/blackjax_b200/csrc/bjx_gemm.h
--- a/blackjax_b200/csrc/bjx_gemm.h
+++ b/blackjax_b200/csrc/bjx_gemm.h
@@ -6,43 +6,35 @@
 
 __host__ __device__ __forceinline__ int plane_stride(int K) { return (K + 7) & ~7; }
 
-__host__ __device__ __forceinline__ float pow2_lift_to(float amax, int e) {
+__host__ __device__ __forceinline__ float pow2_lift(float amax) {
   if (!(amax > 0.f) || amax > 3.0e38f) return 1.f;
   union { float f; uint32_t u; } b;
   b.f = amax;
-  int s = e - ((int)((b.u >> 23) & 0xffu) - 127);
+  int s = 13 - ((int)((b.u >> 23) & 0xffu) - 127);
   s = s < -126 ? -126 : (s > 126 ? 126 : s);
   b.u = (uint32_t)(s + 127) << 23;
   return b.f;
 }
-__host__ __device__ __forceinline__ float pow2_lift(float amax) { return pow2_lift_to(amax, 13); }
-__host__ __device__ __forceinline__ float plane_lift(float stale_max) { return pow2_lift_to(stale_max, 6); }
-constexpr float kPlaneWindowLo = 0.125f;
-constexpr float kPlaneWindowHi = 46340.0f;
 
 struct GemmEpilogue {
   float alpha;
   const float* alpha_dev;
-  const float* x_unscale;
   const float* mat_unscale;
   float beta;
   int has_cin;
   int double_kick;
-  int planes;
-  float* out_unscale;
-  const float* stale_max;
-  float* next_max;
-  float* zero_max;
+  float* out_max;
+  float* clear_max;
   int debug;
 };
 
 struct GemmCall {
-  const uint16_t* x_planes;
+  const float* X;
+  const float* x_max;
   const uint16_t* a_planes;
   float* Y;
   const float* Cin;
-  uint16_t* planes_out;
-  int M, N, K, KP, KP_out;
+  int M, N, K;
   GemmEpilogue epi;
 };
 
```

New measurement: 42.80 million (median of 6 runs). 0.568x the previous value.
